# WujiangXu/AMID

Measured on AMD Instinct MI355X. Metric: train samples/sec, higher is better.
Workload: dtype f32; 1 GPU; cloth_sport_train75-shaped SASRec train step (BASELINE.json configs[1]); batch_per_gpu=256, global_batch=256, seq_len=50, emb_dim=128, hid_dim=32, neg=1, table_rows=894820, unique_rows_last_step=2102, input=HBM-resident batch pool, dropout=on (p=0.5), optimizer=Adam (dense-equivalent lazy rows), graph=True, steps_per_graph=1, parallelism=dp1

## Files before the change

amid_amd/csrc/sasrec_strip.hip:

```cpp
#include "common.h"
#include "rng.h"
#include "strip_gemm.h"
#include "strip_chain.h"
#include "sort_phases.h"
#include "attention_mfma.h"
#include "seq_bwd.h"
#include "scorer_sum.h"
#include <type_traits>

namespace amid {

struct StripQkvArgs {
    const float* x;
    const float* ln_w[2]; const float* ln_b[2];
    const float* w_in[2]; const float* b_in[2];
    float* qn; float* q; float* k; float* v;
    float ln_eps;
};

struct StripOffArgs {
    const float* o; const float* qn;
    const float* w_o[2]; const float* b_o[2]; const float* ln_w[2]; const float* ln_b[2];
    const float* w1[2]; const float* b1[2]; const float* w2[2]; const float* b2[2];
    const unsigned char* tmq;
    float* r; float* y; float* h; float* xo;
    float ln_eps;
    const StepState* st; int train; unsigned spec; float scale; int layer;
};

template <int D, bool XSTORE>
__device__ __forceinline__ void qkv_fwd_chain(const StripQkvArgs& a, const StripGeom& sg, Ring<D>& ring, const StripRow& row, int g,
                                              const StripRegs<D>& X, const ColVec<D>& lw, const ColVec<D>& lb) {
    constexpr int NT = D / 16;
    const GBuf gx(a.x, sg.act_bytes), gqn(a.qn, sg.act_bytes), gq(a.q, sg.act_bytes), gk(a.k, sg.act_bytes), gv(a.v, sg.act_bytes);
    StripRegs<D> Qn, Kr, Vr;
    ColVec<D> bias;
    strip_layernorm<D>(Qn, X, lw, lb, a.ln_eps);
    STRIP_STAMP(3);
    f32x4 acc[NT];
    {
        const float* buf = ring.next();
        STRIP_STAMP(4);
        bias.load(a.b_in[g] + D);
        strip_zero<D>(acc);
        strip_mma<D>(acc, X, buf, [&](int ct, int j) {
            ring.fetch(a.w_in[g] + 2LL * D * D, ct, j);
            if constexpr (XSTORE) store_spread<D>(gx, row, X, ct, j);
            store_spread<D>(gqn, row, Qn, ct, j);
        });
        STRIP_STAMP(5);
        add_bias<D>(acc, bias);
        to_regs<D>(Kr, acc);
        STRIP_STAMP(6);
    }
    {
        const float* buf = ring.next();
        STRIP_STAMP(7);
        bias.load(a.b_in[g] + 2 * D);
        strip_zero<D>(acc);
        strip_mma<D>(acc, X, buf, [&](int ct, int j) { ring.fetch(a.w_in[g], ct, j); store_spread<D>(gk, row, Kr, ct, j); });
        STRIP_STAMP(8);
        add_bias<D>(acc, bias);
        to_regs<D>(Vr, acc);
    }
    {
        const float* buf = ring.next();
        STRIP_STAMP(9);
        bias.load(a.b_in[g]);
        strip_zero<D>(acc);
        strip_mma<D>(acc, Qn, buf, [&](int ct, int j) { store_spread<D>(gv, row, Vr, ct, j); });
        STRIP_STAMP(10);
        add_bias<D>(acc, bias);
        to_regs<D>(Kr, acc);
        strip_store<D>(gq, row, Kr);
        STRIP_STAMP(11);
    }
}

template <int D>
__global__ __launch_bounds__(STRIP_THREADS) void strip_qkv_fwd_kernel(const StripQkvArgs a, const StripGeom sg) {
    extern __shared__ __attribute__((aligned(16))) float smem[];
    STRIP_STAMP(0);
    Ring<D> ring(smem);
    ring.first(a.w_in[strip_domain(blockIdx.x)] + 1LL * D * D);
    const StripTile t = strip_tile(sg, blockIdx.x);
    if (!t.live) { w_ring_wait(); return; }
    const StripRow row = strip_row<D>(sg, t);
    STRIP_STAMP(1);
    StripRegs<D> X;
    ColVec<D> lw, lb;
    strip_load<D>(X, GBuf(a.x, sg.act_bytes), row);
    lw.load(a.ln_w[t.g]); lb.load(a.ln_b[t.g]);
    STRIP_STAMP(2);
    qkv_fwd_chain<D, false>(a, sg, ring, row, t.g, X, lw, lb);
}

struct StripGatherArgs { const float* table; const int* idx; const float* pos[2]; unsigned char* tmq; };

template <int D>
__global__ __launch_bounds__(STRIP_THREADS) void strip_qkv_fwd_gather_kernel(const StripQkvArgs a, const StripGatherArgs ga, const StripGeom sg) {
    extern __shared__ __attribute__((aligned(16))) float smem[];
    Ring<D> ring(smem);
    ring.first(a.w_in[strip_domain(blockIdx.x)] + 1LL * D * D);
    const StripTile t = strip_tile(sg, blockIdx.x);
    if (!t.live) { w_ring_wait(); return; }
    const StripRow row = strip_row<D>(sg, t);
    StripRegs<D> X;
    ColVec<D> lw, lb;
    {
        const int gq = lane_id() >> 4;
        const int id = ga.idx[(long long)t.g * sg.M + row.local];
        const float* __restrict__ trow = ga.table + (long long)id * D;
        const float* __restrict__ prow = ga.pos[t.g] + (long long)(row.local % sg.T) * D;
        const GBuf gtm(ga.tmq, sg.tm_bytes);
        const unsigned tbase = row.ok ? (row.off - 16u * (unsigned)gq) >> 4 : STRIP_OOB;
#pragma unroll
        for (int ct = 0; ct < D / 16; ++ct) {
            const int col = ct * 16 + 4 * gq;
            const float4 tv = ld4_global(trow + col), pv = ld4_global(prow + col);
            float4 x = make_float4(tv.x + pv.x, tv.y + pv.y, tv.z + pv.z, tv.w + pv.w);
            const unsigned bits = (x.x == 0.f ? 1u : 0u) | (x.y == 0.f ? 2u : 0u) | (x.z == 0.f ? 4u : 0u) | (x.w == 0.f ? 8u : 0u);
            if (bits & 1u) x.x = 0.f;
            if (bits & 2u) x.y = 0.f;
            if (bits & 4u) x.z = 0.f;
            if (bits & 8u) x.w = 0.f;
            X.v[ct] = row.ok ? f32x4{x.x, x.y, x.z, x.w} : f32x4{0.f, 0.f, 0.f, 0.f};
            __builtin_amdgcn_raw_buffer_store_b8((unsigned char)bits, gtm.r, row.ok ? (int)(tbase + (unsigned)(ct * 4 + gq)) : (int)STRIP_OOB, 0, 0);
        }
    }
    lw.load(a.ln_w[t.g]); lb.load(a.ln_b[t.g]);
    qkv_fwd_chain<D, false>(a, sg, ring, row, t.g, X, lw, lb);
}

template <int D, bool NEXT, bool SAVE = true>
__global__ __launch_bounds__(STRIP_THREADS) void strip_oproj_ffn_fwd_kernel(const StripOffArgs a, const StripQkvArgs nx, const StripGeom sg) {
    extern __shared__ __attribute__((aligned(16))) float smem[];
    constexpr int NT = D / 16;
    Ring<D> ring(smem);
    ring.first(a.w_o[strip_domain(blockIdx.x)]);
    const StripTile t = strip_tile(sg, blockIdx.x);
    if (!t.live) { w_ring_wait(); return; }
    const StripRow row = strip_row<D>(sg, t);
    const int g = t.g;
    unsigned long long seed = 0; unsigned step = 0;
    if (a.train) { seed = a.st->seed; step = (unsigned)a.st->step; }
    const GBuf gr(a.r, sg.act_bytes), gy(a.y, sg.act_bytes), gh(a.h, sg.act_bytes), gxo(a.xo, sg.act_bytes);
    StripRegs<D> A, R, Y, H;
    StripTm<D> tm;
    ColVec<D> bias, lw, lb;
    strip_load<D>(A, GBuf(a.o, sg.act_bytes), row);
    strip_load<D>(R, GBuf(a.qn, sg.act_bytes), row);
    const bool has_tm = a.tmq != nullptr;
    if (has_tm) strip_tm_load<D>(tm, GBuf(a.tmq, sg.tm_bytes), row);
    bias.load(a.b_o[g]); lw.load(a.ln_w[g]); lb.load(a.ln_b[g]);
    f32x4 acc[NT];
    {
        const float* buf = ring.next();
        strip_zero<D>(acc);
        strip_mma<D>(acc, A, buf, [&](int ct, int j) { ring.fetch(a.w1[g], ct, j); });
        add_bias<D>(acc, bias);
// ... 327 lines not shown
        if (l == 0) strip_store<D>(GBuf(P.a.dx, sg.act_bytes), row, DX);
        DZ = DX;
    }
    STRIP_RSTAMP(13);
    STRIP_STAMP(15);
    w_ring_wait();
}

}

using namespace amid;
using namespace amid_strip_host;

static int make_rider(SortRider& rd, const void* sort_plan, int sort_phase) {
    rd.phase = 0;
    if (sort_plan == nullptr) return AMID_OK;
    if (sort_phase < 1 || sort_phase > 4) return AMID_ERR_ARG;
    rd.plan = *(const SortPlan*)sort_plan;
    rd.phase = sort_phase;
    return AMID_OK;
}

template <auto KERNEL, int DVAL, class... Args>
static int launch_strip_rider(const StripGeom& sg, const SortRider& rd, int extra, void* stream, const Args&... args) {
    if (rd.phase != 0 && strip_lds_bytes<DVAL>() < (rd.plan.g0.bits > 10 ? sizeof(SortScatterLds<OS_BINS_MAX>) : sizeof(SortScatterLds<1024>))) return AMID_ERR_UNSUPPORTED;
    return launch_lds<KERNEL>(2 * sg.tpg + rider_blocks_host(rd) + extra, STRIP_THREADS, strip_lds_bytes<DVAL>(), stream, args..., sg, rd);
}

extern "C" int amid_sas_strip_tile_rows(void) { return STRIP_TILE; }

#ifdef AMID_STRIP_STAMPS
extern "C" int amid_strip_stamps_read(unsigned long long* host) {
    return (int)hipMemcpyFromSymbol(host, HIP_SYMBOL(amid::amid_strip_stamp_buf), sizeof(unsigned long long) * STRIP_STAMP_WAVES * 32);
}
#endif

static void fill_strip_qkv(StripQkvArgs& a, const float* x, const float* const* ln_w, const float* const* ln_b, const float* const* w_in,
                           const float* const* b_in, float ln_eps, float* qn, float* q, float* k, float* v) {
    a.x = x; a.qn = qn; a.q = q; a.k = k; a.v = v; a.ln_eps = ln_eps;
    for (int g = 0; g < 2; ++g) { a.ln_w[g] = ln_w[g]; a.ln_b[g] = ln_b[g]; a.w_in[g] = w_in[g]; a.b_in[g] = b_in[g]; }
}

extern "C" int amid_sas_strip_qkv_fwd_f32(const float* x, const float* const* ln_w, const float* const* ln_b, const float* const* w_in,
                                          const float* const* b_in, float ln_eps, int B, int T, int D, const int* live, float* qn, float* q,
                                          float* k, float* v, void* stream) {
    AMID_CHECK_ARG(x && ln_w && ln_b && w_in && b_in && qn && q && k && v);
    StripQkvArgs a;
    fill_strip_qkv(a, x, ln_w, ln_b, w_in, b_in, ln_eps, qn, q, k, v);
    StripGeom sg;
    if (int e = make_strip_geom(B, T, D, live, &sg)) return e;
    if (D == 128) return launch_strip<strip_qkv_fwd_kernel<128>, 128>(sg, stream, a);
    if (D == 64) return launch_strip<strip_qkv_fwd_kernel<64>, 64>(sg, stream, a);
    return AMID_ERR_UNSUPPORTED;
}

struct StripOffCall {
    const float* o = nullptr; const float* qn = nullptr;
    FamC w_o = nullptr, b_o = nullptr, ln_w = nullptr, ln_b = nullptr, w1 = nullptr, b1 = nullptr, w2 = nullptr, b2 = nullptr;
    const unsigned char* tmq = nullptr; float ln_eps = 0.f;
    int B = 0, T = 0, D = 0; const int* live = nullptr; void* stream = nullptr;
    int layer = 0; const void* step_state = nullptr; int train = 0; float p_drop = 0.f;
    float* r = nullptr; float* y = nullptr; float* h = nullptr; float* xo = nullptr;
    FamC nln_w = nullptr, nln_b = nullptr, nw_in = nullptr, nb_in = nullptr;
    float* nqn = nullptr; float* nq = nullptr; float* nk = nullptr; float* nv = nullptr;
    bool save = true;
    bool next() const { return nln_w != nullptr; }
    bool next_operands() const { return nln_b && nw_in && nb_in && nqn && nq && nk && nv; }
};
#define STRIP_OFF_CALL(c)                                                                                                                       \
    StripOffCall c;                                                                                                                             \
    c.o = o; c.qn = qn; c.w_o = w_o; c.b_o = b_o; c.ln_w = ln_w; c.ln_b = ln_b; c.w1 = w1; c.b1 = b1; c.w2 = w2; c.b2 = b2; c.tmq = tmq;             \
    c.ln_eps = ln_eps; c.B = B; c.T = T; c.D = D; c.live = live; c.stream = stream; c.xo = xo; c.nln_w = nln_w; c.nln_b = nln_b; c.nw_in = nw_in;   \
    c.nb_in = nb_in; c.nqn = nqn; c.nq = nq; c.nk = nk; c.nv = nv

template <int D, bool SAVE>
static int launch_oproj_ffn_fwd(const StripGeom& sg, void* stream, bool next, const StripOffArgs& a, const StripQkvArgs& nx) {
    return next ? launch_strip<strip_oproj_ffn_fwd_kernel<D, true, SAVE>, D>(sg, stream, a, nx)
                : launch_strip<strip_oproj_ffn_fwd_kernel<D, false, SAVE>, D>(sg, stream, a, nx);
}
static int strip_oproj_ffn_fwd(const StripOffCall& c) {
    const bool next = c.next();
    StripOffArgs a;
    a.o = c.o; a.qn = c.qn; a.tmq = c.tmq; a.r = c.r; a.y = c.y; a.h = c.h; a.xo = c.xo; a.ln_eps = c.ln_eps;
    a.st = (const StepState*)c.step_state; a.layer = c.layer;
    const DropoutArgs d = dropout_args(c.train, c.p_drop);
    a.train = d.train; a.spec = d.spec; a.scale = d.scale;
    for (int g = 0; g < 2; ++g) {
        a.w_o[g] = c.w_o[g]; a.b_o[g] = c.b_o[g]; a.ln_w[g] = c.ln_w[g]; a.ln_b[g] = c.ln_b[g];
        a.w1[g] = c.w1[g]; a.b1[g] = c.b1[g]; a.w2[g] = c.w2[g]; a.b2[g] = c.b2[g];
    }
    StripQkvArgs nx = {};
    if (next) fill_strip_qkv(nx, c.save ? c.xo : nullptr, c.nln_w, c.nln_b, c.nw_in, c.nb_in, c.ln_eps, c.nqn, c.nq, c.nk, c.nv);
    StripGeom sg;
    if (int e = make_strip_geom(c.B, c.T, c.D, c.live, &sg)) return e;
    if (c.D == 128) return c.save ? launch_oproj_ffn_fwd<128, true>(sg, c.stream, next, a, nx) : launch_oproj_ffn_fwd<128, false>(sg, c.stream, next, a, nx);
    if (c.D == 64) return c.save ? launch_oproj_ffn_fwd<64, true>(sg, c.stream, next, a, nx) : launch_oproj_ffn_fwd<64, false>(sg, c.stream, next, a, nx);
    return AMID_ERR_UNSUPPORTED;
}

extern "C" int amid_sas_strip_oproj_ffn_fwd_f32(const float* o, const float* qn, const float* const* w_o, const float* const* b_o,
                                                const float* const* ln_w, const float* const* ln_b, const float* const* w1,
                                                const float* const* b1, const float* const* w2, const float* const* b2,
                                                const unsigned char* tmq, float ln_eps, int B, int T, int D, const int* live, int layer,
                                                const void* step_state, int train, float p_drop, float* r, float* y, float* h, float* xo,
                                                const float* const* nln_w, const float* const* nln_b, const float* const* nw_in,
                                                const float* const* nb_in, float* nqn, float* nq, float* nk, float* nv, void* stream) {
    STRIP_OFF_CALL(c); c.layer = layer; c.step_state = step_state; c.train = train; c.p_drop = p_drop; c.r = r; c.y = y; c.h = h;
    AMID_CHECK_ARG(o && qn && w_o && b_o && ln_w && ln_b && w1 && b1 && w2 && b2 && r && y && h && xo && (!train || step_state));
    AMID_CHECK_ARG(!c.next() || c.next_operands());
    return strip_oproj_ffn_fwd(c);
}

extern "C" int amid_sas_strip_infer_supported(int T, int D) { return (T > 0 && (D == 128 || D == 64)) ? 1 : 0; }

extern "C" int amid_sas_strip_qkv_fwd_gather_infer_f32(const float* table, const int* idx_all, const float* pos0, const float* pos1,
                                                       const float* const* ln_w, const float* const* ln_b, const float* const* w_in,
                                                       const float* const* b_in, float ln_eps, int B, int T, int D, const int* live,
                                                       unsigned char* tmq, float* qn, float* q, float* k, float* v, void* stream) {
    AMID_CHECK_ARG(table && idx_all && pos0 && pos1 && ln_w && ln_b && w_in && b_in && tmq && qn && q && k && v && B > 0 && T > 0 && D > 0);
    for (int g = 0; g < 2; ++g) AMID_CHECK_ARG(ln_w[g] && ln_b[g] && w_in[g] && b_in[g]);
    if (!amid_sas_strip_infer_supported(T, D)) return AMID_ERR_UNSUPPORTED;
    StripQkvArgs a;
    fill_strip_qkv(a, nullptr, ln_w, ln_b, w_in, b_in, ln_eps, qn, q, k, v);
    StripGatherArgs ga;
    ga.table = table; ga.idx = idx_all; ga.pos[0] = pos0; ga.pos[1] = pos1; ga.tmq = tmq;
    StripGeom sg;
    if (int e = make_strip_geom(B, T, D, live, &sg)) return e;
    if (D == 128) return launch_strip<strip_qkv_fwd_gather_kernel<128>, 128>(sg, stream, a, ga);
    return launch_strip<strip_qkv_fwd_gather_kernel<64>, 64>(sg, stream, a, ga);
}

extern "C" int amid_sas_strip_oproj_ffn_fwd_infer_f32(const float* o, const float* qn, const float* const* w_o, const float* const* b_o,
                                                      const float* const* ln_w, const float* const* ln_b, const float* const* w1,
                                                      const float* const* b1, const float* const* w2, const float* const* b2,
                                                      const unsigned char* tmq, float ln_eps, int B, int T, int D, const int* live, float* xo,
                                                      const float* const* nln_w, const float* const* nln_b, const float* const* nw_in,
                                                      const float* const* nb_in, float* nqn, float* nq, float* nk, float* nv, void* stream) {
    STRIP_OFF_CALL(c); c.save = false;
    AMID_CHECK_ARG(o && qn && w_o && b_o && ln_w && ln_b && w1 && b1 && w2 && b2 && B > 0 && T > 0 && D > 0);
    AMID_CHECK_ARG(c.next() ? c.next_operands() : xo != nullptr);
    for (int g = 0; g < 2; ++g) {
        AMID_CHECK_ARG(w_o[g] && b_o[g] && ln_w[g] && ln_b[g] && w1[g] && b1[g] && w2[g] && b2[g]);
        AMID_CHECK_ARG(!c.next() || (nln_w[g] && nln_b[g] && nw_in[g] && nb_in[g]));
    }
    if (!amid_sas_strip_infer_supported(T, D)) return AMID_ERR_UNSUPPORTED;
    return strip_oproj_ffn_fwd(c);
}
#undef STRIP_OFF_CALL

struct StripBwdLaunch {
    int B = 0, T = 0, D = 0; const int* live = nullptr;
    const void* sort_plan = nullptr; int sort_phase = 0;
    int mma_bf16 = 0;
    void* stream = nullptr;
};
#define STRIP_BWD_LAUNCH(l) StripBwdLaunch l; l.B = B; l.T = T; l.D = D; l.live = live; l.mma_bf16 = mma_bf16; l.stream = stream
#define STRIP_BWD_RIDER(l) l.sort_plan = sort_plan; l.sort_phase = sort_phase

template <int D, int BF>
static int launch_ffn_bwd(const StripGeom& sg, const SortRider& rd, void* stream, const StripFfnBwdArgs& a) {
    return rd.phase ? launch_strip_rider<strip_ffn_bwd_kernel<D, 2, BF>, D>(sg, rd, 0, stream, a)
                    : launch_strip_rider<strip_ffn_bwd_kernel<D, 0, BF>, D>(sg, rd, 0, stream, a);
}
static int strip_ffn_bwd(const FfnBwdCall& c, const StripBwdLaunch& l) {
    AMID_CHECK_ARG(c.dxo && c.operands());
    const int D = l.D, mma_bf16 = l.mma_bf16;
    if (mma_bf16 && D != 128) return AMID_ERR_UNSUPPORTED;
    StripFfnBwdArgs a;
    fill_ffn_bwd(a, c);
    StripGeom sg;
    if (int e = make_strip_geom(l.B, l.T, D, l.live, &sg)) return e;
    SortRider rd;
    if (int e = make_rider(rd, l.sort_plan, l.sort_phase)) return e;
    if (rd.phase != 0 && rd.phase != 2) return AMID_ERR_UNSUPPORTED;
    if (D == 128) return mma_bf16 == 3 ? launch_ffn_bwd<128, 3>(sg, rd, l.stream, a) : mma_bf16 ? launch_ffn_bwd<128, 1>(sg, rd, l.stream, a)
                                                                                          : launch_ffn_bwd<128, 0>(sg, rd, l.stream, a);
    if (D == 64) return launch_ffn_bwd<64, 0>(sg, rd, l.stream, a);
    return AMID_ERR_UNSUPPORTED;
}

extern "C" int amid_sas_strip_ffn_bwd_f32(const float* dxo, const unsigned char* tmq, const float* h, const float* r, const float* const* ln_w,
                                          const float* const* w1T, const float* const* w2T, const float* const* woT, float ln_eps, int B, int T,
                                          int D, const int* live, int layer, const void* step_state, int train, float p_drop, float* dpre2,
                                          float* dpre1, float* dr, float* d_o, float* ln_part, int mma_bf16, void* stream) {
    AMID_FFN_BWD_CALL(c); STRIP_BWD_LAUNCH(l);
    return strip_ffn_bwd(c, l);
}

extern "C" int amid_sas_strip_ffn_bwd_sort_f32(const float* dxo, const unsigned char* tmq, const float* h, const float* r,
                                               const float* const* ln_w, const float* const* w1T, const float* const* w2T,
                                               const float* const* woT, float ln_eps, int B, int T, int D, const int* live, int layer,
                                               const void* step_state, int train, float p_drop, float* dpre2, float* dpre1, float* dr,
                                               float* d_o, float* ln_part, const void* sort_plan, int sort_phase, int mma_bf16, void* stream) {
    AMID_CHECK_ARG(sort_plan != nullptr);
    AMID_FFN_BWD_CALL(c); STRIP_BWD_LAUNCH(l); STRIP_BWD_RIDER(l);
    return strip_ffn_bwd(c, l);
}

struct StripQkvBwdCall {
    const float* dq = nullptr; const float* dk = nullptr; const float* dv = nullptr; const float* dr = nullptr; const float* x = nullptr;
    FamC ln_w = nullptr, wqT = nullptr, wkT = nullptr, wvT = nullptr;
    float ln_eps = 0.f; float* dx = nullptr; float* ln_part = nullptr;
    const void* step_state = nullptr; int train = 0;
    FfnBwdCall ffn;
    const unsigned char* emb_tmq = nullptr; float emb_p_drop = 0.f;
    const ScorerSum* scorer = nullptr;
};
#define STRIP_QKV_BWD_CALL(c)                                                                                                                   \
    StripQkvBwdCall c;                                                                                                                          \
    c.dq = dq; c.dk = dk; c.dv = dv; c.dr = dr; c.x = x; c.ln_w = ln_w; c.wqT = wqT; c.wkT = wkT; c.wvT = wvT; c.ln_eps = ln_eps;                   \
    c.ln_part = ln_part; c.step_state = step_state; c.train = train
#define STRIP_QKV_BWD_FFN(c)                                                                                                                    \
    c.ffn.tmq = tmq; c.ffn.h = fh; c.ffn.r = fr; c.ffn.ln_w = fln_w; c.ffn.w1T = fw1T; c.ffn.w2T = fw2T; c.ffn.woT = fwoT; c.ffn.layer = flayer;    \
    c.ffn.p_drop = p_drop; c.ffn.dpre2 = fdpre2; c.ffn.dpre1 = fdpre1; c.ffn.dr = fdr; c.ffn.d_o = fd_o; c.ffn.ln_part = fln_part

template <int D, bool FFN, int BF>
static int launch_qkv_bwd(const StripGeom& sg, const SortRider& rd, void* stream, const StripQkvBwdArgs& a, const StripFfnBwdArgs& f, const ScorerSum& ss) {
    if constexpr (FFN && D == 128 && (BF == 3 || BF == 1))
        if (!rd.phase && ss.nblk > 0) return launch_strip_rider<strip_qkv_bwd_kernel<D, FFN, -1, BF>, D>(sg, rd, ss.nblk, stream, a, f, ss);
    return rd.phase ? launch_strip_rider<strip_qkv_bwd_kernel<D, FFN, FFN ? 3 : 4, BF>, D>(sg, rd, ss.nblk, stream, a, f, ss)
                    : launch_strip_rider<strip_qkv_bwd_kernel<D, FFN, 0, BF>, D>(sg, rd, 0, stream, a, f, ss);
}
static int strip_qkv_bwd(const StripQkvBwdCall& c, const StripBwdLaunch& l) {
    AMID_CHECK_ARG(c.dq && c.dk && c.dv && c.dr && c.x && c.ln_w && c.wqT && c.wkT && c.wvT && c.ln_part);
    const int D = l.D, mma_bf16 = l.mma_bf16;
    if (mma_bf16 && D != 128) return AMID_ERR_UNSUPPORTED;
    const bool ffn = c.ffn.h != nullptr;
    FfnBwdCall fc = c.ffn;
    fc.dxo = nullptr; fc.ln_eps = c.ln_eps; fc.step_state = c.step_state; fc.train = c.train;
    AMID_CHECK_ARG(c.emb_tmq == nullptr || (!ffn && (!c.train || c.step_state)));
    AMID_CHECK_ARG(ffn || c.dx);
    AMID_CHECK_ARG(!ffn || fc.operands());
    StripQkvBwdArgs a;
    a.dq = c.dq; a.dk = c.dk; a.dv = c.dv; a.dr = c.dr; a.x = c.x; a.dx = c.dx; a.ln_part = c.ln_part; a.ln_eps = c.ln_eps;
    for (int g = 0; g < 2; ++g) { a.ln_w[g] = c.ln_w[g]; a.wqT[g] = c.wqT[g]; a.wkT[g] = c.wkT[g]; a.wvT[g] = c.wvT[g]; }
    const DropoutArgs ed = dropout_args(c.emb_tmq && c.train, c.emb_p_drop);
    a.emb_tmq = c.emb_tmq; a.emb_st = (const StepState*)c.step_state;
    a.emb_train = ed.train; a.emb_spec = ed.spec; a.emb_scale = ed.scale;
    StripFfnBwdArgs f = {};
    if (ffn) fill_ffn_bwd(f, fc);
    StripGeom sg;
    if (int e = make_strip_geom(l.B, l.T, D, l.live, &sg)) return e;
    SortRider rd;
    if (int e = make_rider(rd, l.sort_plan, l.sort_phase)) return e;
    if (rd.phase != 0 && rd.phase != (ffn ? 3 : 4)) return AMID_ERR_UNSUPPORTED;
    ScorerSum ss = {};
    if (c.scorer != nullptr) {
        if (!(ffn && D == 128 && (mma_bf16 == 3 || mma_bf16 == 1))) return AMID_ERR_UNSUPPORTED;
        ss = *c.scorer;
    }
    void* const st = l.stream;
    if (D == 128 && mma_bf16 == 3) return ffn ? launch_qkv_bwd<128, true, 3>(sg, rd, st, a, f, ss) : launch_qkv_bwd<128, false, 3>(sg, rd, st, a, f, ss);
    if (D == 128 && mma_bf16) return ffn ? launch_qkv_bwd<128, true, 1>(sg, rd, st, a, f, ss) : launch_qkv_bwd<128, false, 1>(sg, rd, st, a, f, ss);
    if (D == 128) return ffn ? launch_qkv_bwd<128, true, 0>(sg, rd, st, a, f, ss) : launch_qkv_bwd<128, false, 0>(sg, rd, st, a, f, ss);
    if (D == 64) return ffn ? launch_qkv_bwd<64, true, 0>(sg, rd, st, a, f, ss) : launch_qkv_bwd<64, false, 0>(sg, rd, st, a, f, ss);
    return AMID_ERR_UNSUPPORTED;
}

extern "C" int amid_sas_strip_qkv_bwd_f32(const float* dq, const float* dk, const float* dv, const float* dr, const float* x,
                                          const float* const* ln_w, const float* const* wqT, const float* const* wkT, const float* const* wvT,
                                          float ln_eps, int B, int T, int D, const int* live, float* dx, float* ln_part,
                                          const unsigned char* tmq, const float* fh, const float* fr, const float* const* fln_w,
                                          const float* const* fw1T, const float* const* fw2T, const float* const* fwoT, int flayer,
                                          const void* step_state, int train, float p_drop, float* fdpre2, float* fdpre1, float* fdr,
                                          float* fd_o, float* fln_part, int mma_bf16, void* stream) {
    STRIP_QKV_BWD_CALL(c); STRIP_QKV_BWD_FFN(c); c.dx = dx; STRIP_BWD_LAUNCH(l);
    return strip_qkv_bwd(c, l);
}

extern "C" int amid_sas_strip_qkv_bwd_sort_f32(const float* dq, const float* dk, const float* dv, const float* dr, const float* x,
                                               const float* const* ln_w, const float* const* wqT, const float* const* wkT,
                                               const float* const* wvT, float ln_eps, int B, int T, int D, const int* live, float* dx,
                                               float* ln_part, const unsigned char* tmq, const float* fh, const float* fr,
                                               const float* const* fln_w, const float* const* fw1T, const float* const* fw2T,
                                               const float* const* fwoT, int flayer, const void* step_state, int train, float p_drop,
                                               float* fdpre2, float* fdpre1, float* fdr, float* fd_o, float* fln_part, const void* sort_plan,
                                               int sort_phase, int mma_bf16, void* stream) {
    AMID_CHECK_ARG(sort_plan != nullptr);
    STRIP_QKV_BWD_CALL(c); STRIP_QKV_BWD_FFN(c); c.dx = dx; STRIP_BWD_LAUNCH(l); STRIP_BWD_RIDER(l);
    return strip_qkv_bwd(c, l);
}

extern "C" int amid_sas_strip_qkv_bwd_sort_scorer_f32(const float* dq, const float* dk, const float* dv, const float* dr, const float* x,
                                                      const float* const* ln_w, const float* const* wqT, const float* const* wkT,
                                                      const float* const* wvT, float ln_eps, int B, int T, int D, const int* live,
                                                      float* ln_part, const unsigned char* tmq, const float* fh, const float* fr,
                                                      const float* const* fln_w, const float* const* fw1T, const float* const* fw2T,
                                                      const float* const* fwoT, int flayer, const void* step_state, int train, float p_drop,
                                                      float* fdpre2, float* fdpre1, float* fdr, float* fd_o, float* fln_part,
                                                      const void* sort_plan, int sort_phase, int mma_bf16, const float* hidg, const float* u,
                                                      const float* items, int NI, int hid, float* dW1, float* db1, float* dW2, float* db2,
                                                      void* stream) {
    AMID_CHECK_ARG(sort_plan != nullptr && fh != nullptr && hidg && u && items && NI > 0 && hid > 0 && dW1 && db1 && dW2 && db2);
    AMID_CHECK_ARG(((((unsigned long long)dW1) | ((unsigned long long)u) | ((unsigned long long)items)) & 15) == 0);
    const ScorerSum ss = scorer_sum_args(hidg, u, items, B, NI, D, hid, dW1, db1, dW2, db2);
    STRIP_QKV_BWD_CALL(c); STRIP_QKV_BWD_FFN(c); c.scorer = &ss; STRIP_BWD_LAUNCH(l); STRIP_BWD_RIDER(l);
    return strip_qkv_bwd(c, l);
}

extern "C" int amid_sas_strip_qkv_bwd_scorer_f32(const float* dq, const float* dk, const float* dv, const float* dr, const float* x,
                                                 const float* const* ln_w, const float* const* wqT, const float* const* wkT,
                                                 const float* const* wvT, float ln_eps, int B, int T, int D, const int* live,
                                                 float* ln_part, const unsigned char* tmq, const float* fh, const float* fr,
                                                 const float* const* fln_w, const float* const* fw1T, const float* const* fw2T,
                                                 const float* const* fwoT, int flayer, const void* step_state, int train, float p_drop,
                                                 float* fdpre2, float* fdpre1, float* fdr, float* fd_o, float* fln_part, int mma_bf16,
                                                 const float* hidg, const float* u, const float* items, int NI, int hid, float* dW1, float* db1,
                                                 float* dW2, float* db2, void* stream) {
    AMID_CHECK_ARG(fh != nullptr && hidg && u && items && NI > 0 && hid > 0 && dW1 && db1 && dW2 && db2);
    AMID_CHECK_ARG(((((unsigned long long)dW1) | ((unsigned long long)u) | ((unsigned long long)items)) & 15) == 0);
    const ScorerSum ss = scorer_sum_args(hidg, u, items, B, NI, D, hid, dW1, db1, dW2, db2);
    STRIP_QKV_BWD_CALL(c); STRIP_QKV_BWD_FFN(c); c.scorer = &ss; STRIP_BWD_LAUNCH(l);
    return strip_qkv_bwd(c, l);
}

extern "C" int amid_sas_strip_qkv_bwd_emb_f32(const float* dq, const float* dk, const float* dv, const float* dr, const float* x,
                                              const float* const* ln_w, const float* const* wqT, const float* const* wkT,
                                              const float* const* wvT, float ln_eps, int B, int T, int D, const int* live, float* dx,
                                              float* ln_part, const unsigned char* emb_tmq, const void* step_state, int train,
                                              float emb_p_drop, const void* sort_plan, int sort_phase, int mma_bf16, void* stream) {
    AMID_CHECK_ARG(emb_tmq != nullptr && dx != nullptr);
    STRIP_QKV_BWD_CALL(c); c.dx = dx; c.emb_tmq = emb_tmq; c.emb_p_drop = emb_p_drop; STRIP_BWD_LAUNCH(l); STRIP_BWD_RIDER(l);
    return strip_qkv_bwd(c, l);
}
#undef AMID_FFN_BWD_CALL
#undef STRIP_QKV_BWD_FFN
#undef STRIP_QKV_BWD_CALL
#undef STRIP_BWD_RIDER
#undef STRIP_BWD_LAUNCH

template <int D> static constexpr size_t seq_bwd_lds_bytes() { return strip_lds_bytes<D>() + (size_t)STRIP_WAVES * ATTN_BWD_LDS_PER_WAVE; }

extern "C" int amid_sas_seq_bwd_supported(int B, int T, int D, int H) {
    return ((D == 128 || D == 64) && H == 8 && T > 0 && T <= 64 && B > 0 && 2LL * B * T * D * 4 <= 0x7FFFFFF0LL) ? 1 : 0;
}

extern "C" int amid_diag_variants(void) {
#ifdef AMID_DIAG_VARIANTS
    return 1;
#else
    return 0;
#endif
}
static int g_seq_bwd_variant = 0;
extern "C" int amid_sas_seq_bwd_variant(int v) {
    const int prev = g_seq_bwd_variant;
    if (v >= 0) g_seq_bwd_variant = v;
    return prev;
}

extern "C" int amid_sas_seq_bwd_f32(int n_layers, const float* dxo, const unsigned char* tmq, const float* const* h, const float* const* r,
                                    const float* const* x, const float* const* q, const float* const* k, const float* const* v,
                                    const float* const* o, const float* const* stats, const float* const* ln1_w,
                                    const float* const* ln2_w, const float* const* wqT, const float* const* wkT, const float* const* wvT,
                                    const float* const* woT, const float* const* w1T, const float* const* w2T, float ln_eps, int B, int T,
                                    int D, int H, const int* live, const void* step_state, int train, float p_drop, float* const* dpre2,
                                    float* const* dpre1, float* const* dr, float* d_o, float* const* dq, float* const* dk, float* const* dv,
                                    float* dx, float* const* ln1_part, float* const* ln2_part, int mma_bf16, void* stream) {
    AMID_CHECK_ARG(n_layers >= 1 && n_layers <= 2 && dxo && h && r && x && q && k && v && o && stats && ln1_w && ln2_w && wqT && wkT && wvT &&
                   woT && w1T && w2T && live && dpre2 && dpre1 && dr && d_o && dq && dk && dv && dx && ln1_part && ln2_part &&
                   (!train || step_state));
    if (!amid_sas_seq_bwd_supported(B, T, D, H)) return AMID_ERR_UNSUPPORTED;
    SeqBwdArgs a = {};
    a.n_layers = n_layers;
    for (int l = 0; l < n_layers; ++l) {
        SeqBwdLayer& P = a.L[l];
        AMID_CHECK_ARG(h[l] && r[l] && x[l] && q[l] && k[l] && v[l] && o[l] && stats[l] && dpre2[l] && dpre1[l] && dr[l] && dq[l] && dk[l] &&
                       dv[l] && ln1_part[l] && ln2_part[l]);
        for (int g = 0; g < 2; ++g) {
            const int i = 2 * l + g;
            AMID_CHECK_ARG(ln1_w[i] && ln2_w[i] && wqT[i] && wkT[i] && wvT[i] && woT[i] && w1T[i] && w2T[i]);
        }
        FfnBwdCall fc;
        fc.dxo = l + 1 == n_layers ? dxo : nullptr; fc.tmq = tmq; fc.h = h[l]; fc.r = r[l]; fc.ln_w = ln2_w + 2 * l; fc.w1T = w1T + 2 * l;
        fc.w2T = w2T + 2 * l; fc.woT = woT + 2 * l; fc.ln_eps = ln_eps; fc.layer = l; fc.step_state = step_state; fc.train = train; fc.p_drop = p_drop;
        fc.dpre2 = dpre2[l]; fc.dpre1 = dpre1[l]; fc.dr = dr[l]; fc.d_o = d_o; fc.ln_part = ln2_part[l];
        fill_ffn_bwd(P.f, fc);
        P.a.dq = dq[l]; P.a.dk = dk[l]; P.a.dv = dv[l]; P.a.dr = dr[l]; P.a.x = x[l]; P.a.dx = l == 0 ? dx : nullptr;
        P.a.ln_part = ln1_part[l]; P.a.ln_eps = ln_eps;
        for (int g = 0; g < 2; ++g) {
            P.a.ln_w[g] = ln1_w[2 * l + g]; P.a.wqT[g] = wqT[2 * l + g]; P.a.wkT[g] = wkT[2 * l + g]; P.a.wvT[g] = wvT[2 * l + g];
        }
        AttnArgs& at = P.at;
        at.q = q[l]; at.k = k[l]; at.v = v[l]; at.o = const_cast<float*>(o[l]); at.stats = const_cast<float*>(stats[l]);
        at.d_o = d_o; at.dq = dq[l]; at.dk = dk[l]; at.dv = dv[l];
        at.B = B; at.T = T; at.D = D; at.H = H; at.causal = 1; at.layer = l;
        at.scale = sqrtf(1.0f / (float)(D / H));
        at.st = (const StepState*)step_state;
        const DropoutArgs ad = dropout_args(train, p_drop);
        at.train = ad.train; at.thr16 = ad.spec; at.dscale = ad.scale;
        at.stagger_from = -1;
    }
    StripGeom sg;
    if (int e = make_strip_geom(B, T, D, live, &sg)) return e;
    if (g_seq_bwd_variant == 2 || T <= 32 || D != 128) {
        const int rc = launch_seqn_bwd(a, sg, D, mma_bf16, stream);
        if (rc != AMID_ERR_UNSUPPORTED || T <= 32 || D != 128) return rc;
    }
    return mma_bf16 ? launch_lds<seq_bwd_kernel<128, true>>(B, STRIP_THREADS, seq_bwd_lds_bytes<128>(), stream, a, sg)
                    : launch_lds<seq_bwd_kernel<128, false>>(B, STRIP_THREADS, seq_bwd_lds_bytes<128>(), stream, a, sg);
}
```

amid_amd/csrc/sasrec_strip_px.hip:

```cpp
#include "common.h"
#include "rng.h"
#include "strip_gemm.h"
#include "strip_chain.h"
#include "seq_fwd.h"
#include "seq_bwd.h"
#include "seqn_parts.h"
#include "sort_phases.h"

namespace amid {

constexpr int PXB_WPS = 4, PXB_NS = 2, PXB_NW = PXB_WPS * PXB_NS, PXB_THREADS = 64 * PXB_NW;
template <int D> constexpr size_t pxb_lds_floats() {
    return (size_t)3 * (D * D / 2) + (size_t)PXB_WPS * XpStrip<D>::FLOATS + 2 * PXB_NW * 16 + (size_t)PXB_WPS * 2 * D;
}

struct PxbRow { unsigned off_own, phys; int local; bool ok; };
template <int D>
__device__ __forceinline__ PxbRow pxb_row(const StripGeom& sg, const StripTile& t, int si, int c0) {
    PxbRow r;
    int v = t.v0 + si * 16 + (lane_id() & 15);
    r.ok = v < t.nv;
    if (!r.ok) v = t.v0;
    if (sg.live != nullptr) {
        const int s = v / sg.T;
        r.local = sg.live[t.s0 + s] * sg.T + (v - s * sg.T);
    } else {
        r.local = v;
    }
    r.phys = (unsigned)t.g * (unsigned)sg.M + (unsigned)r.local;
    r.off_own = r.ok ? r.phys * (unsigned)(D * 4) + 16u * (unsigned)(lane_id() >> 4) + (unsigned)c0 * 64u : STRIP_OOB;
    return r;
}

template <int NCT>
__device__ __forceinline__ void pxb_row_sums(float* __restrict__ stat, int si, int part, float s1, float s2, float& t1, float& t2) {
    const int m = lane_id() & 15, gq = lane_id() >> 4;
    s1 = row_sum4(s1); s2 = row_sum4(s2);
    if (gq == 0) {
        lds_st1(stat + (si * PXB_NS + part) * 16 + m, s1);
        lds_st1(stat + (PXB_NW + si * PXB_NS + part) * 16 + m, s2);
    }
    lds_barrier();
    t1 = 0.f; t2 = 0.f;
#pragma unroll
    for (int p = 0; p < PXB_NS; ++p) {
        t1 += *(__attribute__((address_space(3))) float*)(stat + (si * PXB_NS + p) * 16 + m);
        t2 += *(__attribute__((address_space(3))) float*)(stat + (PXB_NW + si * PXB_NS + p) * 16 + m);
    }
}

template <int D, int NCT>
__device__ __forceinline__ void pxb_ln_partials(float* __restrict__ scratch, int si, int c0, const PartRegs<NCT>& dgam, const PartRegs<NCT>& dbet) {
    const int lane = lane_id();
    float* mine = scratch + si * 2 * D;
#pragma unroll
    for (int c = 0; c < NCT; ++c) {
        f32x4 a, b;
#pragma unroll
        for (int r = 0; r < 4; ++r) { a[r] = col_sum16(dgam.v[c][r]); b[r] = col_sum16(dbet.v[c][r]); }
        if ((lane & 15) == 0) {
            lds_st4(mine + (c0 + c) * 16 + 4 * (lane >> 4), a);
            lds_st4(mine + D + (c0 + c) * 16 + 4 * (lane >> 4), b);
        }
    }
}
template <int D>
__device__ __forceinline__ void pxb_ln_partials_out(const float* __restrict__ scratch, float* __restrict__ part) {
    for (int e = threadIdx.x; e < 2 * D; e += PXB_THREADS)
        part[e] = (scratch[e] + scratch[2 * D + e]) + (scratch[4 * D + e] + scratch[6 * D + e]);
}

template <int D, int NCT, class Ring>
__device__ __forceinline__ void pxb_ffn_bwd_chain(const StripFfnBwdArgs& a, const float* __restrict__ ln_stat, const StripGeom& sg, Ring& ring,
                                                  const PxbRow& row, int g, int si, int part, int c0, PartRegs<NCT>& DZ, float* __restrict__ xps,
                                                  float* __restrict__ stat, float* __restrict__ lnsc, const unsigned short* __restrict__ wnext) {
    const int lane = lane_id(), gq = lane >> 4;
    const GBuf gp2(a.dpre2, sg.act_bytes), gp1(a.dpre1, sg.act_bytes), gdr(a.dr, sg.act_bytes), gdo(a.d_o, sg.act_bytes);
    PartRegs<NCT> P, Hs, Rs, gam;
    part_load<NCT>(Hs, GBuf(a.h, sg.act_bytes), row.off_own);
    part_load<NCT>(Rs, GBuf(a.r, sg.act_bytes), row.off_own);
    part_cols<NCT>(gam, a.ln_w[g], c0);
    float mean = 0.f, rstd = 0.f;
    if (ln_stat != nullptr && row.ok) { mean = ln_stat[(long long)row.phys * 4 + 2]; rstd = ln_stat[(long long)row.phys * 4 + 3]; }
    if (a.tmq != nullptr) {
        const GBuf gtm(a.tmq, sg.tm_bytes);
        const unsigned tbase = row.ok ? row.phys * (unsigned)(D / 4) + (unsigned)c0 * 4u : STRIP_OOB;
        const int sh = 8 * gq;
#pragma unroll
        for (int c = 0; c < NCT; ++c) {
            const unsigned bits = (unsigned)__builtin_amdgcn_raw_buffer_load_b32(gtm.r, (int)(tbase + 4 * c), 0, 0) >> sh;
            DZ.v[c][0] = (bits & 1u) ? 0.f : DZ.v[c][0];
            DZ.v[c][1] = (bits & 2u) ? 0.f : DZ.v[c][1];
            DZ.v[c][2] = (bits & 4u) ? 0.f : DZ.v[c][2];
            DZ.v[c][3] = (bits & 8u) ? 0.f : DZ.v[c][3];
        }
    }
    P = DZ;
    if (a.train) {
        const uint4 rr2 = rng_call(a.st->seed, (unsigned long long)row.local * D >> 7, site_id(g, a.layer, SITE_FFN2), (unsigned)a.st->step);
        part_dropout<NCT>(P, rr2, c0, a.spec, a.scale, (row.local * D) & 127);
    }
    xp_write<NCT>(xps, c0, P);
    f32x4 acc[NCT];
    {
        ring.next();
        seqn_product_xp<D, NCT>(acc, xps, ring, (const unsigned short*)a.w1T[g], c0, [&](int ct, int j) { part_spread<NCT>(gp2, row.off_own, P, ct, j, 1); });
#pragma unroll
        for (int c = 0; c < NCT; ++c)
#pragma unroll
            for (int r = 0; r < 4; ++r) P.v[c][r] = Hs.v[c][r] > 0.f ? acc[c][r] * a.scale : 0.f;
    }
    lds_barrier();
    xp_write<NCT>(xps, c0, P);
    PartRegs<NCT> DR, dgam, dbet;
    {
        ring.next();
        seqn_product_xp<D, NCT>(acc, xps, ring, (const unsigned short*)a.woT[g], c0, [&](int ct, int j) { part_spread<NCT>(gp1, row.off_own, P, ct, j, 1); });
        if (ln_stat == nullptr) {
            float sm = 0.f;
#pragma unroll
            for (int c = 0; c < NCT; ++c) sm += (Rs.v[c][0] + Rs.v[c][1]) + (Rs.v[c][2] + Rs.v[c][3]);
            float tot, dummy;
            pxb_row_sums<NCT>(stat, si, part, sm, 0.f, tot, dummy);
            mean = tot * (1.0f / D);
            float q = 0.f;
#pragma unroll
            for (int c = 0; c < NCT; ++c)
#pragma unroll
                for (int r = 0; r < 4; ++r) { const float d = Rs.v[c][r] - mean; q = fmaf(d, d, q); }
            lds_barrier();
            float qt;
            pxb_row_sums<NCT>(stat, si, part, q, 0.f, qt, dummy);
            rstd = 1.0f / sqrtf(qt * (1.0f / D) + a.ln_eps);
            lds_barrier();
        }
        float s1 = 0.f, s2 = 0.f;
#pragma unroll
        for (int c = 0; c < NCT; ++c) {
#pragma unroll
            for (int r = 0; r < 4; ++r) {
                const float dy = acc[c][r] + DZ.v[c][r];
                const float xh = (Rs.v[c][r] - mean) * rstd;
                float gy = gam.v[c][r] * dy;
                asm volatile("" : "+v"(gy));
                s1 += gy;
                s2 = fmaf(gy, xh, s2);
                float dg = dy * xh;
                asm volatile("" : "+v"(dg));
                dgam.v[c][r] = dg;
                dbet.v[c][r] = dy;
                DR.v[c][r] = gy;
            }
        }
        float t1, t2;
        pxb_row_sums<NCT>(stat, si, part, s1, s2, t1, t2);
        const float c1 = t1 * (1.0f / D), c2 = t2 * (1.0f / D);
#pragma unroll
        for (int c = 0; c < NCT; ++c)
#pragma unroll
            for (int r = 0; r < 4; ++r) {
                const float xh = (Rs.v[c][r] - mean) * rstd;
                DR.v[c][r] = rstd * (DR.v[c][r] - c1 - xh * c2);
            }
    }
    xp_write<NCT>(xps, c0, DR);
    {
        ring.next();
        seqn_product_xp<D, NCT>(acc, xps, ring, wnext, c0, [&](int ct, int j) { part_spread<NCT>(gdr, row.off_own, DR, ct, j, 1); });
#pragma unroll
        for (int c = 0; c < NCT; ++c) P.v[c] = acc[c];
        part_store<NCT>(gdo, row.off_own, P);
    }
    pxb_ln_partials<D, NCT>(lnsc, si, c0, dgam, dbet);
}

template <int D, int RIDER>
__global__ __launch_bounds__(PXB_THREADS) void strip_ffn_bwd_px_kernel(const StripFfnBwdArgs a, const float* __restrict__ ln_stat, const StripGeom sg,
                                                                       const SortRider rd) {
    extern __shared__ __attribute__((aligned(16))) float smem[];
    constexpr int NCT = D / 16 / PXB_NS;
    int bid = blockIdx.x;
    if constexpr (RIDER != 0) {
        if (bid < rd.plan.nblk) { if (threadIdx.x < SORT_THREADS) sort_phase_ct<RIDER>(rd.plan, bid, smem); return; }
        bid -= rd.plan.nblk;
    }
    const int w = wave_id(), part = w / PXB_WPS, si = w % PXB_WPS, c0 = part * NCT;
    const int g = strip_domain(bid);
    SeqRing3<D, PXB_NW> ring(smem);
    ring.first((const unsigned short*)a.w2T[g]);
    const StripTile t = strip_tile(sg, bid);
    if (!t.live) { zero_slot<D>(a.ln_part, t.slot); w_ring_wait(); return; }
    float* const xps = smem + 3 * SeqRing3<D, PXB_NW>::SLAB + si * XpStrip<D>::FLOATS;
    float* const stat = smem + 3 * SeqRing3<D, PXB_NW>::SLAB + PXB_WPS * XpStrip<D>::FLOATS;
    float* const lnsc = stat + 2 * PXB_NW * 16;
    const PxbRow row = pxb_row<D>(sg, t, si, c0);
    PartRegs<NCT> DZ;
    part_load<NCT>(DZ, GBuf(a.dxo, sg.act_bytes), row.off_own);
    pxb_ffn_bwd_chain<D, NCT>(a, ln_stat, sg, ring, row, g, si, part, c0, DZ, xps, stat, lnsc, (const unsigned short*)a.woT[g]);
    w_ring_wait();
    __syncthreads();
    pxb_ln_partials_out<D>(lnsc, a.ln_part + (long long)t.slot * 2 * D);
}

}

using namespace amid;
using namespace amid_strip_host;

extern "C" int amid_sas_strip_ffn_bwd_px_f32(const float* dxo, const unsigned char* tmq, const float* h, const float* r, const float* const* ln_w,
                                             const float* const* w1T, const float* const* w2T, const float* const* woT, float ln_eps, int B, int T,
                                             int D, const int* live, int layer, const void* step_state, int train, float p_drop, float* dpre2,
                                             float* dpre1, float* dr, float* d_o, float* ln_part, const float* ln_stat, const void* sort_plan,
                                             int sort_phase, void* stream) {
    AMID_FFN_BWD_CALL(c);
    AMID_CHECK_ARG(c.dxo && c.operands());
    if (D != 128) return AMID_ERR_UNSUPPORTED;
    if (train && p_drop > 0.f && spec_bits(drop_spec(p_drop)) != 1) return AMID_ERR_UNSUPPORTED;
    StripGeom sg;
    if (int e = make_strip_geom(B, T, D, live, &sg)) return e;
    StripFfnBwdArgs a;
    fill_ffn_bwd(a, c);
    SortRider rd;
    rd.phase = 0;
    if (sort_plan != nullptr) {
        if (sort_phase != 2) return AMID_ERR_UNSUPPORTED;
        rd.plan = *(const SortPlan*)sort_plan;
        rd.phase = sort_phase;
    }
    constexpr size_t lds = pxb_lds_floats<128>() * sizeof(float);
    static_assert(lds >= sizeof(SortScatterLds<OS_BINS_MAX>), "the rider's scatter fits the head of the allocation");
    if (rd.phase != 0) return launch_lds<strip_ffn_bwd_px_kernel<128, 2>>(2 * sg.tpg + rd.plan.nblk, PXB_THREADS, lds, stream, a, ln_stat, sg, rd);
    return launch_lds<strip_ffn_bwd_px_kernel<128, 0>>(2 * sg.tpg, PXB_THREADS, lds, stream, a, ln_stat, sg, rd);
}
#undef AMID_FFN_BWD_CALL
```

amid_amd/engine.py:

```python
from __future__ import annotations

import ctypes
import types
from dataclasses import dataclass
from typing import Dict, List, Optional, Tuple

import torch

from ._lib import lib, ptr_array

from .engine_dp import DataParallelMixin, HipMergeBackend
from .engine_graph import GraphMixin
from .engine_io import InputMixin
from .engine_topk import TopkMixin
from .plan import (DR_HEADS, SASREC_HEADS, SASREC_LN_EPS, SASREC_P_DROP, FlatParams, SasrecPlan, Shape,
                   sasrec_dense_names)

SASREC_FAMILIES = (("ln1_w", "attention_layernorms.{l}.weight"), ("ln1_b", "attention_layernorms.{l}.bias"),
                   ("w_in", "attention_layers.{l}.in_proj_weight"), ("b_in", "attention_layers.{l}.in_proj_bias"),
                   ("w_o", "attention_layers.{l}.out_proj.weight"), ("b_o", "attention_layers.{l}.out_proj.bias"),
                   ("ln2_w", "forward_layernorms.{l}.weight"), ("ln2_b", "forward_layernorms.{l}.bias"),
                   ("w1", "forward_layers.{l}.conv1.weight"), ("b1", "forward_layers.{l}.conv1.bias"),
                   ("w2", "forward_layers.{l}.conv2.weight"), ("b2", "forward_layers.{l}.conv2.bias"))
QKV_FAMILIES = tuple(n for n, _ in SASREC_FAMILIES[:4])
# ... 58 lines not shown
        self._push_step_state()
        self.plans: Dict[Tuple[int, int, int, bool], SasrecPlan] = {}
        self.grad_scale = 1.0
        self.opt_bank, self._banks = 0, {}
        torch.cuda.synchronize(self.device)
        self._ptr_cache: Dict[str, object] = {}

    @property
    def s(self) -> int:
        return self.stream.cuda_stream

    def sync(self) -> None:
        self.join_sort()
        self.stream.synchronize()

    def _push_step_state(self) -> None:
        L = lib()
        host = (ctypes.c_ubyte * self._st_bytes)()
        L.call("amid_step_state_pack", ctypes.addressof(host), self.seed, self.step, self.hyper["lr"], self.hyper["beta1"],
               self.hyper["beta2"], self.hyper["eps"])
        with torch.cuda.stream(self.stream):
            self.step_state.copy_(torch.frombuffer(bytearray(host), dtype=torch.uint8), non_blocking=False)

    @staticmethod
    def rank_seed(seed: int, rank: int) -> int:
        return (int(seed) + 0x9E3779B97F4A7C15 * int(rank)) & 0x7FFFFFFFFFFFFFFF

    def set_step(self, step: int, seed: Optional[int] = None) -> None:
        self.step = int(step)
        if seed is not None:
            self.seed = int(seed)
        self._push_step_state()

    def set_lr(self, lr: float) -> None:
        self.hyper["lr"] = float(lr)
        self._push_step_state()

    def _ensure_opt_state(self) -> None:
        if self.table_m is None:
            self.table_m = torch.zeros_like(self.table)
            self.table_v = torch.zeros_like(self.table)
            self.table_last = torch.zeros(self.n_rows, dtype=torch.int32, device=self.device)
            torch.cuda.synchronize(self.device)

    def select_optimizer(self, k: int, lr: Optional[float] = None) -> None:
        if k == self.opt_bank:
            if lr is not None and lr != self.hyper["lr"]:
                self.set_lr(lr)
            return
        self.flush_table()
        self.sync()
        fp = self.dense
        self._banks[self.opt_bank] = dict(m=fp.m, v=fp.v, tm=self.table_m, tv=self.table_v, tl=self.table_last, st=self.step_state,
                                          step=self.step, lr=self.hyper["lr"], seed=self.seed)
        b = self._banks.get(k)
        if b is None:
            b = dict(m=torch.zeros_like(fp.m), v=torch.zeros_like(fp.v), tm=None, tv=None, tl=None,
                     st=torch.empty(self._st_bytes, dtype=torch.uint8, device=self.device), step=0,
                     lr=self.hyper["lr"] if lr is None else float(lr), seed=self.seed + 0x9E3779B9 * k)
        fp.m, fp.v, self.table_m, self.table_v, self.table_last = b["m"], b["v"], b["tm"], b["tv"], b["tl"]
        self.step_state, self.step, self.seed = b["st"], b["step"], b["seed"]
        self.hyper["lr"] = b["lr"] if lr is None else float(lr)
        self.opt_bank = k
        self._push_step_state()
        torch.cuda.synchronize(self.device)

    def _graph_key(self) -> Tuple[int, int]:
        return (self.opt_bank, self.dr_mode if self.dr else 0)

    def plan(self, B: int, T: int, NI: int, need_grad: bool) -> SasrecPlan:
        key = (B, T, NI, need_grad)
        if key not in self.plans:
            inc = getattr(self, "inc_bs", 0)
            if (2 * T if inc else T) > self.Tpos:
                raise ValueError(f"sequence length {T} exceeds pos_emb size {self.Tpos}" + (" / 2 (isInC)" if inc else ""))
            self.plans[key] = self.PLAN_CLS(self, Shape(B, T, NI, 2 * T if inc else 0), need_grad)
            torch.cuda.synchronize(self.device)
        return self.plans[key]

    def _pp(self, fmt: str, buf: Optional[torch.Tensor] = None, extra: int = 0):
        return self._cached((fmt, 0 if buf is None else buf.data_ptr(), extra),
                            lambda: ptr_array([self.dense.ptr(fmt.format(d=d), buf, extra) for d in (1, 2)]))

    def _wT(self, layer: int, which: int):
        bf = self._bf16_bwd
        p3 = self._p3_bwd
        return self._cached(("wT16x3" if p3 else "wT16" if bf else "wT", layer, which), lambda: ptr_array(
            [(self.wT16x3 if p3 else self.wT16 if bf else self.wT)[layer, g, which].data_ptr() for g in (0, 1)]))

    def _cached(self, key, build):
        c = self._ptr_cache.get(key)
        if c is None:
            c = self._ptr_cache[key] = build()
        return c

    def _fams(self):
        fp = self.dense
        return self._cached("fams", lambda: {n: ptr_array([fp.ptr(f"sac{d}." + fmt.format(l=l)) for l in (0, 1) for d in (1, 2)])
                                             for n, fmt in SASREC_FAMILIES})

    def _lay(self):
        return self._cached("lay", lambda: [{n: self._pp("sac{d}." + fmt.format(l=l)) for n, fmt in SASREC_FAMILIES} for l in (0, 1)])

    def _pos(self):
        fp = self.dense
        return self._cached("pos", lambda: dict(pos0=fp.ptr("sac1.pos_emb.weight"), pos1=fp.ptr("sac2.pos_emb.weight")))

    def _scorer(self, names=("w1", "b1", "w2", "b2"), grad: bool = False):
        fp = self.dense
        return self._cached(("scorer", names, grad), lambda: dict(zip(names, (
            fp.ptr("predictModule.fc." + n, fp.grad if grad else None) for n in ("0.weight", "0.bias", "2.weight", "2.bias")))))

    def _last_ln(self, names=("ln_w", "ln_b")):
        return self._cached(("last_ln", names), lambda: dict(zip(names, (self._pp("sac{d}.last_layernorm.weight"),
                                                                          self._pp("sac{d}.last_layernorm.bias")))))

    def _wT_fams(self, bf16: bool):
        buf = self.wT16 if bf16 else self.wT
        return self._cached(("wT_fams", bool(bf16)), lambda: {
            n: ptr_array([buf[l, g, j].data_ptr() for l in (0, 1) for g in (0, 1)]) for j, n in enumerate(("wqT", "wkT", "wvT", "woT", "w1T", "w2T"))})

    def _wT_lists(self):
        def build():
            fp, D, src, dst = self.dense, self.D, [], []
            for l in (0, 1):
                for g in (0, 1):
                    pre = f"sac{g + 1}"
                    src += [fp.ptr(f"{pre}.attention_layers.{l}.in_proj_weight", None, j * D * D) for j in range(3)]
                    src += [fp.ptr(f"{pre}.attention_layers.{l}.out_proj.weight"), fp.ptr(f"{pre}.forward_layers.{l}.conv1.weight"),
                            fp.ptr(f"{pre}.forward_layers.{l}.conv2.weight")]
                    dst += [self.wT[l, g, w].data_ptr() for w in range(6)]
            return ptr_array(src), ptr_array(dst), len(src)
        return self._cached("wT_lists", build)

    @staticmethod
    def _seq_ptrs(pl: SasrecPlan):
        if not hasattr(pl, "seq_ptrs"):
            pa = lambda ts: ptr_array([t.data_ptr() for t in ts])
            pl.seq_ptrs = dict(x_in=pa(pl.x[:2]), qn=pa(pl.qn), q=pa(pl.q), k=pa(pl.k), v=pa(pl.v), o=pa(pl.o), stats=pa(pl.stats), r=pa(pl.r),
                               y=pa(pl.y), h=pa(pl.h))
        return pl.seq_ptrs

    @staticmethod
    def _seq_grad_ptrs(pl: SasrecPlan):
        if not hasattr(pl, "seq_grad_ptrs"):
            pa = lambda ts: ptr_array([t.data_ptr() for t in ts])
            pl.seq_grad_ptrs = dict(dpre2=pa(pl.dpre2), dpre1=pa(pl.dpre1), dr=pa(pl.dr), dq=pa(pl.dq_l), dk=pa(pl.dk_l), dv=pa(pl.dv_l),
                                    ln1_part=pa(pl.ln1_part_s), ln2_part=pa(pl.ln2_part_s))
        return pl.seq_grad_ptrs

    _bf16_bwd = False
    _p3_bwd = False
    BWD_SPLIT = True

    def enqueue_prepare(self, pl: SasrecPlan, sparse: bool, bump_step: bool = False, defer_sort: bool = False) -> None:
        L, s, shp = lib(), self.s, pl.shape
        with_live = bool(bump_step and getattr(pl, "strip", False) and not self.itc_bs)
        pl.live_packed = with_live
        pl.compact = bool(with_live and sparse and self.compact_ok(pl))
        pl.riding = bool(bump_step and sparse and defer_sort and self.SORT_RIDERS and getattr(pl, "strip", False) and not pl.compact
                         and not self._seq_backward(pl)
                         and (shp.n_idx + 2047) // 2048 <= 2 * shp.Tenc and self._sort_plan(pl) is not None)
        pl.chain = bool(bump_step and sparse and defer_sort and self.SORT_CHAIN and not pl.riding and not pl.compact
                        and shp.n_idx <= lib().value("amid_sort_chain_max_indices") and self.n_rows <= (1 << 20) and self._sort_plan(pl) is not None)
        ent = self.input_pool(pl)
        self._bf16_as_f32 = False
        if self.compute == "bf16" and self.BF16_FOLD and bump_step and shp.B <= self.BF16_FOLD_MAX_B:
            self._bf16_as_f32 = True
            if not (ent is not None and sparse and defer_sort and with_live and self._tail2_ok(pl)):
                self._bf16_as_f32 = False
            else:
                pl.riding = False
        pl.tail2 = bool(ent is not None and bump_step and sparse and defer_sort and with_live and self._tail2_ok(pl))
        pl.gather_on_fwd = False
        pl.prepared = False
        if pl.tail2:
            pool, phase = ent
            self._ensure_opt_state()
            head = (pool.data_ptr(), pool.stride(0), pool.shape[0], phase, pl.in_pack.data_ptr(), pl.in_words, shp.B, shp.T,
                    shp.NI - 1, self.n_rows, pl.idx_all.data_ptr(), pl.idx_c.data_ptr(), pl.row_c.data_ptr(), pl.live.data_ptr(), pl.err.data_ptr(),
                    self.table.data_ptr(), self.table_m.data_ptr(), self.table_v.data_ptr(), self.table_last.data_ptr(), self.D,
                    self.step_state.data_ptr(), self._sort_plan_c(pl))
            pl.gather_on_fwd = bool(self.GATHER_ON_FWD and self._fwd_on_pieces(pl, shp.B, shp.Tenc) and self._p3_bwd_for(pl) and shp.T == shp.Tenc)
            slabs = self.pool_slabs(pl)
            pl.prepared = bool(self.PREPARED_POOL and slabs is not None and getattr(self, "_in_train_step", False) and self.compute != "bf16")
            if pl.prepared:
                w = (None, 0, 0, None, None)
                if pl.gather_on_fwd:
                    src, w16 = self._w16_images(3)
                    w = (src, 24, 3, w16.data_ptr(), self._wT16x3_buf().data_ptr())
                L.call("amid_step_head_prepared_f32", *head, slabs[0].data_ptr(), slabs[0].stride(0), *w, s)
            elif pl.gather_on_fwd:
                src, w16 = self._w16_images(3)
                L.call("amid_step_head_w16_f32", *head, src, 24, 3, w16.data_ptr(), self._wT16x3_buf().data_ptr(), s)
            else:
                L.call("amid_step_head_f32", *head, s)
            self.step += 1
            pl.compact, pl.riding, pl.chain = True, not pl.prepared, False
            self._sort_owed = False
            return
        if ent is not None:
            pool, phase = ent
            if not bump_step:
                raise ValueError("an input pool advances with the step counter: enqueue_prepare(bump_step=True) only")
            if with_live:
                L.call("amid_pack_indices_pool_live", pool.data_ptr(), pool.stride(0), pool.shape[0], phase, pl.in_pack.data_ptr(),
                       pl.in_words, shp.B, shp.T, shp.NI - 1, self.n_rows, pl.idx_all.data_ptr(), pl.err.data_ptr(),
                       self.step_state.data_ptr(), pl.live.data_ptr(), s)
            else:
                L.call("amid_pack_indices_pool", pool.data_ptr(), pool.stride(0), pool.shape[0], phase, pl.in_pack.data_ptr(),
                       pl.in_words, shp.B, shp.T, shp.NI - 1, self.n_rows, pl.idx_all.data_ptr(), pl.err.data_ptr(),
                       self.step_state.data_ptr(), s)
            self.step += 1
            if sparse and (pl.riding or pl.chain):
                self._sort_owed = False
            elif sparse:
                self.ev_idx.record(self.stream)
                self._sort_owed = bool(defer_sort)
                if not defer_sort:
                    self.enqueue_sort(pl)
            return
        if with_live:
            L.call("amid_pack_indices_live", pl.in_i_node.data_ptr(), pl.in_neg.data_ptr(), pl.in_seq_d1.data_ptr(), pl.in_seq_d2.data_ptr(),
                   shp.B, shp.T, shp.NI - 1, self.n_rows, pl.idx_all.data_ptr(), pl.err.data_ptr(),
                   self.step_state.data_ptr() if bump_step else None, pl.domain.data_ptr(), pl.live.data_ptr(), s)
        else:
            L.call("amid_pack_indices", pl.in_i_node.data_ptr(), pl.in_neg.data_ptr(), pl.in_seq_d1.data_ptr(), pl.in_seq_d2.data_ptr(),
                   shp.B, shp.T, shp.NI - 1, self.n_rows, pl.idx_all.data_ptr(), pl.err.data_ptr(),
                   self.step_state.data_ptr() if bump_step else None, s)
        if bump_step:
            self.step += 1
        if sparse and (pl.riding or pl.chain):
            self._sort_owed = False
        elif sparse:
            self.ev_idx.record(self.stream)
            self._sort_owed = bool(defer_sort)
            if not defer_sort:
                self.enqueue_sort(pl)

    def enqueue_sort(self, pl: SasrecPlan) -> None:
        L, shp = lib(), pl.shape
        self.side.wait_event(self.ev_idx)
        if getattr(pl, "compact", False):
            L.call("amid_sort_unique_rows_i32", pl.idx_c.data_ptr(), pl.row_c.data_ptr(), pl.n_compact, self.n_rows, pl.sort_ws.data_ptr(),
                   pl.pos_sorted.data_ptr(), pl.uniq_ids.data_ptr(), pl.seg_off.data_ptr(), pl.seg_of.data_ptr(), pl.n_uniq.data_ptr(),
                   self.side.cuda_stream)
        else:
            L.call("amid_sort_unique_i32", pl.idx_all.data_ptr(), shp.n_idx, self.n_rows, pl.sort_ws.data_ptr(), pl.pos_sorted.data_ptr(),
                   pl.uniq_ids.data_ptr(), pl.seg_off.data_ptr(), pl.seg_of.data_ptr(), pl.n_uniq.data_ptr(), self.side.cuda_stream)
        self.ev_sorted.record(self.side)
        self._sort_pending = True
        self._sort_owed = False

    def _wgrad_mode(self, D: int) -> int:
        if D != 128:
            return 0
        if self.BF16_WGRAD and getattr(self, "_bf16_bwd", False):
            return 1
        if self._bf16_as_f32 and self.BF16_WGRAD and self.BF16_FWD_ONE and getattr(self, "_wgrad_one", False):
            return 4
        return {"9": 2, "6": 3}.get(self.WGRAD_SPLIT, 0)

    def join_sort(self) -> None:
        if getattr(self, "_sort_pending", False):
            self.stream.wait_event(self.ev_sorted)
            self._sort_pending = False

    SORT_RIDERS = True
    BF16_FOLD = True
    BF16_FOLD_MAX_B = 1 << 30
    BF16_FWD_ONE = True
    _bf16_as_f32 = False

    def _ceff(self) -> str:
        return "f32" if self._bf16_as_f32 else self.compute
    FOLD_SHORT = True
    SORT_CHAIN = False
    BF16_WGRAD = True
    WGRAD_SPLIT = "6"
    FWD_SPLIT = True
    SEQ_BACKWARD = "auto"

    def _seq_backward(self, pl: SasrecPlan) -> bool:
        if not getattr(pl, "seq_bwd", False) or self.itc_bs or self.SEQ_BACKWARD in ("0", False):
            return False
        if self.SEQ_BACKWARD in ("1", True):
            return True
        n_cu = torch.cuda.get_device_properties(self.device).multi_processor_count
        if pl.shape.Tenc <= 32:
            if self.FOLD_SHORT and pl.shape.Tenc > 16 and self.D == 128 and self._folded_step_shape(pl):
                return False
            return pl.shape.B <= n_cu
        if self.D != 128:
            return False
        if self._folded_step_shape(pl):
            return False
        return n_cu < pl.shape.B <= 2 * n_cu

    def _sort_plan(self, pl: SasrecPlan):
        if not hasattr(pl, "_sort_plan_buf"):
            L = lib()
            buf = (ctypes.c_ubyte * L.value("amid_sort_plan_bytes"))()
            rc = L._fn["amid_sort_plan_pack"](ctypes.addressof(buf), pl.idx_all.data_ptr(), None, pl.shape.n_idx, self.n_rows,
                                              pl.sort_ws.data_ptr(), pl.pos_sorted.data_ptr(), pl.uniq_ids.data_ptr(), pl.seg_off.data_ptr(),
                                              pl.seg_of.data_ptr(), pl.n_uniq.data_ptr())
            pl._sort_plan_buf = buf if rc == 0 else None
# ... 392 lines not shown
                pl.du_raw.copy_(pl.du_raw_g[:, ex.rank * B:(ex.rank + 1) * B])
                for d in (1, 2):
                    for name in ("trans_nn.weight", "trans_nn.bias", "trans_bs.weight", "trans_bs.bias"):
                        self.dense.view(f"itc_d{d}.{name}", G).mul_(1.0 / ex.world)
            du = pl.du_raw
        L.call("amid_lnmean_bwd_f32", pl.x[2].data_ptr(), du.data_ptr(), fp.ptr("sac1.last_layernorm.weight"),
               fp.ptr("sac2.last_layernorm.weight"), B, T, D, SASREC_LN_EPS, pl.dxbuf.data_ptr(), pl.last_part.data_ptr(), s)

    def _scorer_fwd(self, pl: SasrecPlan, head: str, items: int, p1, p2, with_loss: bool) -> None:
        shp, fp = pl.shape, self.dense
        lib().call("amid_scorer_fwd_f32", pl.u.data_ptr(), items, fp.ptr(f"{head}.fc.0.weight"), fp.ptr(f"{head}.fc.0.bias"),
                   fp.ptr(f"{head}.fc.2.weight"), fp.ptr(f"{head}.fc.2.bias"), pl.labels.data_ptr() if with_loss else None,
                   pl.domain.data_ptr() if with_loss else None, shp.B, shp.NI, self.D, self.hid, p1.data_ptr(), p2.data_ptr(),
                   pl.dp1.data_ptr() if with_loss else None, pl.dp2.data_ptr() if with_loss else None,
                   pl.loss_part.data_ptr() if with_loss else None, self.s)

    def _scorer_bwd(self, pl: SasrecPlan, head: str, items: int, ditems: int, p1, p2, dp1, dp2, part, accumulate: int) -> None:
        shp, fp = pl.shape, self.dense
        lib().call("amid_scorer_bwd_f32", pl.u.data_ptr(), items, fp.ptr(f"{head}.fc.0.weight"), fp.ptr(f"{head}.fc.0.bias"),
                   fp.ptr(f"{head}.fc.2.weight"), fp.ptr(f"{head}.fc.2.bias"), p1.data_ptr(), p2.data_ptr(), dp1.data_ptr(), dp2.data_ptr(),
                   shp.B, shp.NI, self.D, self.hid, pl.du.data_ptr(), ditems, part.data_ptr(), accumulate, self.s)

    def _enqueue_head_itc_fwd(self, pl: SasrecPlan, items: int, with_loss: bool) -> None:
        self._enqueue_user_vectors(pl)
        self._scorer_fwd(pl, "predictModule", items, pl.p1, pl.p2, with_loss)

    def _enqueue_head_itc_bwd(self, pl: SasrecPlan, items: int, ditems: int) -> None:
        self._scorer_bwd(pl, "predictModule", items, ditems, pl.p1, pl.p2, pl.dp1, pl.dp2, pl.sc_part, 0)
        self._enqueue_user_vectors_bwd(pl)

    def _enqueue_head_dr_fwd(self, pl: SasrecPlan, items: int, with_loss: bool) -> None:
        L, shp = lib(), pl.shape
        self._enqueue_user_vectors(pl)
        self._scorer_fwd(pl, "predictModule", items, pl.p1, pl.p2, False)
        self._scorer_fwd(pl, "predict_ips", items, pl.ips1, pl.ips2, False)
        self._scorer_fwd(pl, "predict_gfunc", items, pl.g1, pl.g2, False)
        if with_loss:
            pa = lambda a, b: ptr_array([a.data_ptr(), b.data_ptr()])
            L.call("amid_dr_loss_f32", pa(pl.p1, pl.p2), pa(pl.ips1, pl.ips2), pa(pl.g1, pl.g2), pl.labels.data_ptr(), pl.domain.data_ptr(),
                   pl.in_ob.data_ptr(), self.dr_mode, self.dr_e_w, shp.B, shp.NI, pa(pl.dp1, pl.dp2), pa(pl.dips1, pl.dips2),
                   pa(pl.dg1, pl.dg2), pl.dr_loss_part.data_ptr(), self.s)

    def _enqueue_head_dr_bwd(self, pl: SasrecPlan, items: int, ditems: int) -> None:
        self._scorer_bwd(pl, "predictModule", items, ditems, pl.p1, pl.p2, pl.dp1, pl.dp2, pl.sc_part, 0)
        self._scorer_bwd(pl, "predict_ips", items, ditems, pl.ips1, pl.ips2, pl.dips1, pl.dips2, pl.sc_part_ips, 1)
        self._scorer_bwd(pl, "predict_gfunc", items, ditems, pl.g1, pl.g2, pl.dg1, pl.dg2, pl.sc_part_g, 1)
        self._enqueue_user_vectors_bwd(pl)

    def _enqueue_scorers_fused(self, pl: SasrecPlan, items: int, ditems: int, tr_src, tr_dst, n_tr: int) -> None:
        shp, fp = pl.shape, self.dense
        heads = DR_HEADS if self.dr else DR_HEADS[:1]
        outs = [(pl.p1, pl.p2, pl.dp1, pl.dp2, pl.sc_part)]
        if self.dr:
            outs += [(pl.ips1, pl.ips2, pl.dips1, pl.dips2, pl.sc_part_ips), (pl.g1, pl.g2, pl.dg1, pl.dg2, pl.sc_part_g)]
        pa = lambda seq: ptr_array(list(seq))
        lib().call("amid_scorer_multi_fwd_bwd_f32", pl.u.data_ptr(), items, pa(fp.ptr(f"{h}.fc.0.weight") for h in heads),
                   pa(fp.ptr(f"{h}.fc.0.bias") for h in heads), pa(fp.ptr(f"{h}.fc.2.weight") for h in heads),
                   pa(fp.ptr(f"{h}.fc.2.bias") for h in heads), len(heads), pl.labels.data_ptr(), pl.domain.data_ptr(),
                   pl.in_ob.data_ptr() if self.dr else None, self.dr_mode if self.dr else 0, self.dr_e_w, shp.B, shp.NI, self.D, self.hid,
                   pa(o[0].data_ptr() for o in outs), pa(o[1].data_ptr() for o in outs), pa(o[2].data_ptr() for o in outs),
                   pa(o[3].data_ptr() for o in outs), pl.loss_part.data_ptr(), pl.dr_loss_part.data_ptr() if self.dr else None,
                   pl.du.data_ptr(), ditems, pa(o[4].data_ptr() for o in outs), tr_src, tr_dst, n_tr, self.s)

    def _head_io(self, pl: SasrecPlan, items: int, ditems: int):
        shp = pl.shape
        return dict(x=pl.x[2].data_ptr(), items=items, labels=pl.labels.data_ptr(), domain_id=pl.domain.data_ptr(), B=shp.B, T=shp.Tenc, NI=shp.NI,
                    D=self.D, hid=self.hid, eps=SASREC_LN_EPS, u=pl.u.data_ptr(), p1=pl.p1.data_ptr(), p2=pl.p2.data_ptr(), dp1=pl.dp1.data_ptr(),
                    dp2=pl.dp2.data_ptr(), loss_part=pl.loss_part.data_ptr(), dx=pl.dxbuf.data_ptr(), ditems=ditems,
                    ln_part=pl.last_part.data_ptr(), stream=self.s)

    def enqueue_backward(self, pl: SasrecPlan, train: bool) -> None:
        L, s, shp, D = lib(), self.s, pl.shape, self.D
        B, T, NI, M = shp.B, shp.Tenc, shp.NI, shp.M
        st = self.step_state.data_ptr()
        tr = 1 if train else 0
        fp = self.dense
        tr_src, tr_dst, n_tr = self._wT_lists()
        self._bf16_bwd = bool(self._ceff() == "bf16" and pl.strip)
        self._p3_bwd = self._p3_bwd_for(pl)
        bf = 3 if self._p3_bwd else 1 if self._bf16_bwd else 0
        if self._bf16_as_f32 and self._p3_bwd:
            bf = 1
        if self._bf16_bwd:
            if not hasattr(self, "wT16"):
                self.wT16 = torch.empty(2, 2, 6, D * D, dtype=torch.bfloat16, device=self.device)
            L.call("amid_sas_weights_bf16", tr_src, n_tr, D, 1, self.wT16.data_ptr(), s)
        if self._p3_bwd:
            if not getattr(pl, "wT16x3_written", False):
                L.call("amid_sas_weights_bf16_planes", tr_src, n_tr, D, 1, 3, self._wT16x3_buf().data_ptr(), s)
            pl.wT16x3_written = False
        items = pl.xg.data_ptr() + 4 * 2 * shp.Mi * D
        ditems = pl.dxg.data_ptr() + 4 * 2 * shp.Mi * D
        if (self.dr or self.itc_bs) and getattr(self, "_fuse_scorers", False):
            self._enqueue_scorers_fused(pl, items, ditems, tr_src, tr_dst, n_tr)
            self._enqueue_user_vectors_bwd(pl)
        elif self.dr:
            L.call("amid_transpose_weights_f32", tr_src, tr_dst, n_tr, D, s)
            self._enqueue_head_dr_bwd(pl, items, ditems)
        elif self.itc_bs:
            L.call("amid_transpose_weights_f32", tr_src, tr_dst, n_tr, D, s)
            self._enqueue_head_itc_bwd(pl, items, ditems)
        elif getattr(pl, "head_done", False):
            pl.head_done = False
        elif getattr(self, "_fuse_head", False) and getattr(pl, "tail2", False) and getattr(self, "_live_fwd", False) and self._live_list(pl) is not None:
            L.call_named("amid_head_fwd_bwd_own_vec_f32", self._last_ln(), self._scorer(), self._head_io(pl, items, ditems),
                         hidg=self._hidg(pl).data_ptr(), tr_src=None, tr_dst=None, n_tr=0)
        elif getattr(self, "_fuse_head", False):
            L.call_named("amid_head_fwd_bwd_own_f32" if getattr(self, "_live_fwd", False) and self._live_list(pl) is not None else "amid_head_fwd_bwd_f32",
                         self._last_ln(), self._scorer(), self._head_io(pl, items, ditems), sc_part=pl.sc_part.data_ptr(), tr_src=tr_src,
                         tr_dst=tr_dst, n_tr=n_tr)
        else:
            L.call_named("amid_head_bwd_f32", self._last_ln(), self._scorer(), x=pl.x[2].data_ptr(), u=pl.u.data_ptr(), items=items,
                         p1=pl.p1.data_ptr(), p2=pl.p2.data_ptr(), dp1=pl.dp1.data_ptr(), dp2=pl.dp2.data_ptr(), B=B, T=T, NI=NI, D=D,
                         hid=self.hid, eps=SASREC_LN_EPS, dx=pl.dxbuf.data_ptr(), ditems=ditems, ln_part=pl.last_part.data_ptr(),
                         sc_part=pl.sc_part.data_ptr(), tr_src=tr_src, tr_dst=tr_dst, n_tr=n_tr, stream=s)
        def ffn_bwd_args(l):
            return (pl.tmq.data_ptr(), pl.h[l].data_ptr(), pl.r[l].data_ptr(), self._pp(f"sac{{d}}.forward_layernorms.{l}.weight"),
                    self._wT(l, 4), self._wT(l, 5), self._wT(l, 3))

        lv = self._live_list(pl)
        live_attn = lv is not None and bool(lib().value("amid_attn_live_supported", T, D, self.H, 1))

        def attn_bwd(l):
            if live_attn:
                L.call("amid_attn_bwd_live_f32", pl.q[l].data_ptr(), pl.k[l].data_ptr(), pl.v[l].data_ptr(), pl.o[l].data_ptr(),
                       pl.stats[l].data_ptr(), pl.d_o.data_ptr(), B, T, D, self.H, 1, l, st, tr, SASREC_P_DROP, pl.dq_l[l].data_ptr(),
                       pl.dk_l[l].data_ptr(), pl.dv_l[l].data_ptr(), lv, s)
                return
            L.call("amid_attn_bwd_rows_f32", pl.q[l].data_ptr(), pl.k[l].data_ptr(), pl.v[l].data_ptr(), pl.o[l].data_ptr(),
                   pl.stats[l].data_ptr(), pl.d_o.data_ptr(), None, B, T, D, self.H, 1, l, st, tr, SASREC_P_DROP, pl.dq_l[l].data_ptr(),
                   pl.dk_l[l].data_ptr(), pl.dv_l[l].data_ptr(), self._own_rows(pl), s)

        dom = self._own_rows(pl)
        live = dom is not None and pl.live_rows
        tm, h1, r1, lnw1, w1T1, w2T1, woT1 = ffn_bwd_args(1)
        tm, h0, r0, lnw0, w1T0, w2T0, woT0 = ffn_bwd_args(0)
        dx_in = (pl.dx0 if self.inc_bs else pl.dxg).data_ptr()
        seq = bool(pl.strip and lv is not None and live and live_attn and self._seq_backward(pl))
        pl.seq_bwd_used = seq
        if seq:
            sv = self._seq_ptrs(pl)
            L.call_named("amid_sas_seq_bwd_f32", sv, self._seq_grad_ptrs(pl), self._fams(), self._wT_fams(bf), n_layers=2, dxo=pl.dxbuf.data_ptr(),
                         tmq=tm, x=sv["x_in"], ln_eps=SASREC_LN_EPS, B=B, T=T, D=D, H=self.H, live=lv, step_state=st, train=tr,
                         p_drop=SASREC_P_DROP, d_o=pl.d_o.data_ptr(), dx=dx_in, mma_bf16=bf, stream=s)
        elif pl.strip:
            ln1p, ln2p = pl.ln1_part, pl.ln2_part
            riding = getattr(pl, "riding", False)
            sfx = "_sort" if riding else ""
            t2 = getattr(pl, "tail2", False)
            plan_addr = (self._sort_plan_c(pl) if t2 else self._sort_plan(pl)) if riding else None
            ride = lambda ph: (plan_addr, ph) if riding else ()
            L.call(f"amid_sas_strip_ffn_bwd{sfx}_f32", pl.dxbuf.data_ptr(), tm, h1, r1, lnw1, w1T1, w2T1, woT1, SASREC_LN_EPS, B, T, D, lv, 1, st, tr,
                   SASREC_P_DROP, pl.dpre2[1].data_ptr(), pl.dpre1[1].data_ptr(), pl.dr[1].data_ptr(), pl.d_o.data_ptr(), ln2p[1].data_ptr(),
                   *ride(2), bf, s)
            attn_bwd(1)
            if t2:
                mid = ("amid_sas_strip_qkv_bwd_sort_scorer_f32", dict(sort_plan=plan_addr, sort_phase=3)) if riding else ("amid_sas_strip_qkv_bwd_scorer_f32", {})
                L.call_named(mid[0], self._scorer(("dW1", "db1", "dW2", "db2"), grad=True), **mid[1],
                             dq=pl.dq_l[1].data_ptr(), dk=pl.dk_l[1].data_ptr(), dv=pl.dv_l[1].data_ptr(), dr=pl.dr[1].data_ptr(),
                             x=pl.x[1].data_ptr(), ln_w=self._pp("sac{d}.attention_layernorms.1.weight"), wqT=self._wT(1, 0), wkT=self._wT(1, 1),
                             wvT=self._wT(1, 2), ln_eps=SASREC_LN_EPS, B=B, T=T, D=D, live=lv, ln_part=ln1p[1].data_ptr(), tmq=tm, fh=h0, fr=r0,
                             fln_w=lnw0, fw1T=w1T0, fw2T=w2T0, fwoT=woT0, flayer=0, step_state=st, train=tr, p_drop=SASREC_P_DROP,
                             fdpre2=pl.dpre2[0].data_ptr(), fdpre1=pl.dpre1[0].data_ptr(), fdr=pl.dr[0].data_ptr(), fd_o=pl.d_o.data_ptr(),
                             fln_part=ln2p[0].data_ptr(), mma_bf16=bf, hidg=self._hidg(pl).data_ptr(),
                             u=pl.u.data_ptr(), items=items, NI=NI, hid=self.hid, stream=s)
            else:
                L.call(f"amid_sas_strip_qkv_bwd{sfx}_f32", pl.dq_l[1].data_ptr(), pl.dk_l[1].data_ptr(), pl.dv_l[1].data_ptr(), pl.dr[1].data_ptr(),
                       pl.x[1].data_ptr(), self._pp("sac{d}.attention_layernorms.1.weight"), self._wT(1, 0), self._wT(1, 1), self._wT(1, 2),
                       SASREC_LN_EPS, B, T, D, lv, None, ln1p[1].data_ptr(), tm, h0, r0, lnw0, w1T0, w2T0, woT0, 0, st, tr, SASREC_P_DROP,
                       pl.dpre2[0].data_ptr(), pl.dpre1[0].data_ptr(), pl.dr[0].data_ptr(), pl.d_o.data_ptr(), ln2p[0].data_ptr(), *ride(3), bf, s)
            attn_bwd(0)
            if t2:
                L.call("amid_sas_strip_qkv_bwd_emb_f32", pl.dq_l[0].data_ptr(), pl.dk_l[0].data_ptr(), pl.dv_l[0].data_ptr(), pl.dr[0].data_ptr(),
                       pl.x[0].data_ptr(), self._pp("sac{d}.attention_layernorms.0.weight"), self._wT(0, 0), self._wT(0, 1), self._wT(0, 2),
                       SASREC_LN_EPS, B, T, D, lv, dx_in, ln1p[0].data_ptr(), pl.tmq.data_ptr(), st, tr, SASREC_P_DROP, plan_addr, 4 if riding else 0, bf, s)
            else:
                L.call(f"amid_sas_strip_qkv_bwd{sfx}_f32", pl.dq_l[0].data_ptr(), pl.dk_l[0].data_ptr(), pl.dv_l[0].data_ptr(), pl.dr[0].data_ptr(),
                       pl.x[0].data_ptr(), self._pp("sac{d}.attention_layernorms.0.weight"), self._wT(0, 0), self._wT(0, 1), self._wT(0, 2),
                       SASREC_LN_EPS, B, T, D, lv, dx_in, ln1p[0].data_ptr(), None, None, None, None, None, None, None, 0, None, 0, 0.0, None,
                       None, None, None, None, *ride(4), bf, s)
        else:
            rows, suf, rpt = ("_rows", pl.rt_suffix_v, pl.rpt_v) if live else ("", pl.rt_suffix, pl.rpt)
            ln1p, ln2p = (pl.ln1_part_v, pl.ln2_part_v) if live else (pl.ln1_part, pl.ln2_part)
            hint = (dom, B, T) if live else ()
            L.call(f"amid_sas_ffn_bwd{rows}_f32" + suf, pl.dxbuf.data_ptr(), tm, h1, r1, lnw1, w1T1, w2T1, woT1, SASREC_LN_EPS, M, D, rpt, 1, st, tr,
                   SASREC_P_DROP, pl.dpre2[1].data_ptr(), pl.dpre1[1].data_ptr(), pl.dr[1].data_ptr(), pl.d_o.data_ptr(),
                   ln2p[1].data_ptr(), self.mma_bf16, *hint, s)
            attn_bwd(1)
            L.call(f"amid_sas_qkv_ffn_bwd{rows}_f32" + suf, pl.dq_l[1].data_ptr(), pl.dk_l[1].data_ptr(), pl.dv_l[1].data_ptr(), pl.dr[1].data_ptr(),
                   pl.x[1].data_ptr(), self._pp("sac{d}.attention_layernorms.1.weight"), self._wT(1, 0), self._wT(1, 1), self._wT(1, 2),
                   SASREC_LN_EPS, M, D, rpt, pl.dxbuf.data_ptr(), ln1p[1].data_ptr(), tm, h0, r0, lnw0, w1T0, w2T0, woT0, 0, st, tr,
                   SASREC_P_DROP, pl.dpre2[0].data_ptr(), pl.dpre1[0].data_ptr(), pl.dr[0].data_ptr(), pl.d_o.data_ptr(),
                   ln2p[0].data_ptr(), self.mma_bf16, *hint, s)
            attn_bwd(0)
            L.call(f"amid_sas_qkv_bwd{rows}_f32" + suf, pl.dq_l[0].data_ptr(), pl.dk_l[0].data_ptr(), pl.dv_l[0].data_ptr(), pl.dr[0].data_ptr(),
                   pl.x[0].data_ptr(), self._pp("sac{d}.attention_layernorms.0.weight"), self._wT(0, 0), self._wT(0, 1), self._wT(0, 2),
                   SASREC_LN_EPS, M, D, rpt, dx_in, ln1p[0].data_ptr(), self.mma_bf16, *hint, s)
        dy, xx = [], []
        for l in (0, 1):
            dy += [pl.dq_l[l].data_ptr(), pl.dk_l[l].data_ptr(), pl.dv_l[l].data_ptr(), pl.dr[l].data_ptr(), pl.dpre1[l].data_ptr(),
                   pl.dpre2[l].data_ptr()]
            xx += [pl.qn[l].data_ptr(), pl.x[l].data_ptr(), pl.x[l].data_ptr(), pl.o[l].data_ptr(), pl.y[l].data_ptr(), pl.h[l].data_ptr()]
        t2 = bool(getattr(pl, "tail2", False) and pl.strip and not seq)
        if t2:
            if getattr(pl, "lnstat_fwd", False):
                for l in (0, 1):
                    xx[6 * l + 0], xx[6 * l + 4] = pl.x[l].data_ptr(), pl.r[l].data_ptr()
                self._wgrad_one = True
                try:
                    wmode = self._wgrad_mode(D)
                finally:
                    self._wgrad_one = False
                wg = ("amid_sas_wgrad_rows_sort_ln_f32", dict(sort_plan=self._sort_plan_c(pl))) if pl.riding else ("amid_sas_wgrad_rows_ln_f32", {})
                L.call_named(wg[0], self._fams(), dy=ptr_array(dy), x=ptr_array(xx), n_layers=2, M=M, D=D,
                             splits=pl.splits, w_part=ptr_array([pl.w_part[0].data_ptr(), pl.w_part[1].data_ptr()]),
                             b_part=ptr_array([pl.b_part[0].data_ptr(), pl.b_part[1].data_ptr()]), row_domain=self._own_rows(pl), B=B, T=T,
                             mma_bf16=wmode, ln_stat=self._ln_stat(pl)[1], stream=s, **wg[1])
            elif not pl.riding:
                L.call("amid_sas_wgrad_rows_f32", ptr_array(dy), ptr_array(xx), 2, M, D, pl.splits,
                       ptr_array([pl.w_part[0].data_ptr(), pl.w_part[1].data_ptr()]), ptr_array([pl.b_part[0].data_ptr(), pl.b_part[1].data_ptr()]),
                       self._own_rows(pl), B, T, self._wgrad_mode(D), s)
            else:
                L.call("amid_sas_wgrad_rows_sort_f32", ptr_array(dy), ptr_array(xx), 2, M, D, pl.splits,
                       ptr_array([pl.w_part[0].data_ptr(), pl.w_part[1].data_ptr()]), ptr_array([pl.b_part[0].data_ptr(), pl.b_part[1].data_ptr()]),
                       self._own_rows(pl), B, T, self._wgrad_mode(D), self._sort_plan_c(pl), s)
            self._enqueue_grad_tail(pl, live, seq)
            return
        L.call("amid_sas_wgrad_rows_f32", ptr_array(dy), ptr_array(xx), 2, M, D, pl.splits, ptr_array([pl.w_part[0].data_ptr(), pl.w_part[1].data_ptr()]),
               ptr_array([pl.b_part[0].data_ptr(), pl.b_part[1].data_ptr()]), self._own_rows(pl), B, T,
               self._wgrad_mode(D), s)
        if getattr(pl, "riding", False):
            L.call("amid_embed_bwd_sort_f32", (pl.dx0 if self.inc_bs else pl.dxg).data_ptr(), pl.tmq.data_ptr(), B, T, D, pl.pos_splits,
                   pl.dpos_part.data_ptr(), st, tr, SASREC_P_DROP, dom if live else None, self._sort_plan(pl), 5, s)
        elif live:
            L.call("amid_embed_bwd_rows_f32", (pl.dx0 if self.inc_bs else pl.dxg).data_ptr(), pl.tmq.data_ptr(), B, T, D, pl.pos_splits,
                   pl.dpos_part.data_ptr(), st, tr, SASREC_P_DROP, dom, s)
        else:
            L.call("amid_embed_bwd_f32", (pl.dx0 if self.inc_bs else pl.dxg).data_ptr(), pl.tmq.data_ptr(), B, T, D, pl.pos_splits,
                   pl.dpos_part.data_ptr(), st, tr, SASREC_P_DROP, s)
        if self.inc_bs:
            G = self.dense.grad
            head = (pl.dpos_part.data_ptr(), pl.pos_splits, pl.xg.data_ptr(), pl.dx0.data_ptr(), pl.inc_gate.data_ptr(), pl.inc_S.data_ptr(),
                    pl.inc_sw.data_ptr(), self._pp("inc_d{d}.trans_nn.weight"), self._pp("inc_d{d}.trans_nn.bias"),
                    self._pp("inc_d{d}.trans_bs.weight"), B, shp.T, D)
            outs = (pl.inc_dZ.data_ptr(), pl.inc_dS.data_ptr(), pl.inc_rows.data_ptr(), self._pp("inc_d{d}.trans_nn.weight", G),
                    self._pp("inc_d{d}.trans_nn.bias", G), self._pp("inc_d{d}.trans_bs.weight", G), self._pp("inc_d{d}.trans_bs.bias", G),
                    pl.dxg.data_ptr(), s)
            if getattr(pl, "inc_world", 1) > 1:
                ex = self._inc_exchange(pl)
                shard = (self.inc_bs, ex.rank * B)
                L.call("amid_inc_bwd_shard_f32", *head, *shard, 1, 1.0 / ex.world, *outs)
                self._coll(lambda: ex.all_reduce_dense(pl.inc_dZ))
                L.call("amid_inc_bwd_shard_f32", *head, *shard, 2, 1.0 / ex.world, *outs)
            else:
                L.call("amid_inc_bwd_f32", *head, *outs)
        self._enqueue_grad_tail(pl, live, seq)

    def _enqueue_grad_tail(self, pl: SasrecPlan, live: bool = False, seq: bool = False) -> None:
        L, s, shp = lib(), self.s, pl.shape
        if getattr(self, "_sort_owed", False):
            self.ev_idx.record(self.stream)
            self.enqueue_sort(pl)
        self.join_sort()
        blk = (pl.red_blk_s if seq else getattr(pl, "red_blk_v", None) if live else None) or pl.red_blk
        ent, n_ent, ent_max = ((pl.red_entries_s, pl.red_n_s, pl.red_max_s) if seq else (pl.red_entries_v, pl.red_n_v, pl.red_max_v) if live
                               else (pl.red_entries, pl.red_n, pl.red_max))
        pk = getattr(self, "_tail_pack", None)
        pl.spans_done = False
        if getattr(pl, "tail2", False) and not getattr(self, "_in_train_step", False):
            ent_t, n_ent_t, blk_t = self._tail2_table(pl)
            fp = self.dense
            head = (pl.dxg.data_ptr(), pl.pos_sorted.data_ptr(), pl.seg_off.data_ptr(), pl.seg_of.data_ptr(), pl.n_compact, self.D,
                    pl.seg_ws.data_ptr())
            mid = (ent_t.data_ptr(), n_ent_t, blk_t[0].data_ptr(), blk_t[1], pl.live.data_ptr(), shp.B, shp.Tenc,
                   fp.ptr("sac1.pos_emb.weight", fp.grad), fp.ptr("sac2.pos_emb.weight", fp.grad))
            if self.FUSED_OPT:
                left_lo = fp.slots["predictModule.fc.0.weight"][0]
                dense = (fp.grad.data_ptr(), fp.numel, left_lo, fp.numel, pl.uniq_ids.data_ptr(), pl.n_uniq.data_ptr(), pl.n_compact)
                if pk is not None:
                    from .dist import packed_rows
                    send, umax, with_dense = pk
                    id_rows, rows = packed_rows(umax, self.D)
                    L.call("amid_grad_tail_live_dp1_f32", *head, send.data_ptr() + 4 * id_rows * self.D, *mid, *dense, umax, self.n_rows,
                           send.data_ptr(), send.data_ptr() + 4 * rows * self.D if with_dense else None, pl.err.data_ptr(),
                           pl.tail_ticket.data_ptr(), s)
                else:
                    L.call("amid_grad_tail_live_dp1_f32", *head, pl.uniq_grad.data_ptr(), *mid, *dense, 0, 0, None, None, None,
                           pl.tail_ticket.data_ptr(), s)
            elif pk is not None:
                from .dist import packed_rows
                send, umax, with_dense = pk
                id_rows, rows = packed_rows(umax, self.D)
                L.call("amid_grad_tail_live_dp_f32", *head, send.data_ptr() + 4 * id_rows * self.D, *mid, pl.uniq_ids.data_ptr(),
                       pl.n_uniq.data_ptr(), umax, self.n_rows, send.data_ptr(), self.dense.grad.data_ptr() if with_dense else None,
                       send.data_ptr() + 4 * rows * self.D if with_dense else None, self.dense.numel if with_dense else 0,
                       pl.err.data_ptr(), s)
            else:
                L.call("amid_grad_tail_live_dp_f32", *head, pl.uniq_grad.data_ptr(), *mid, None, None, 0, 0, None, None, None, 0, None, s)
            pl.spans_done = True
            return
        pl.opt_done = False
        if getattr(pl, "tail2", False) and self.FUSED_OPT and self.table_m is not None and not self.dr:
            ent_t, n_ent_t, blk_t = self._tail2_table(pl)
            fp = self.dense
            left_lo = fp.slots["predictModule.fc.0.weight"][0]
            L.call("amid_grad_tail_opt_f32", pl.dxg.data_ptr(), pl.pos_sorted.data_ptr(), pl.seg_off.data_ptr(), pl.seg_of.data_ptr(), pl.n_compact,
                   self.D, pl.seg_ws.data_ptr(), pl.uniq_grad.data_ptr(), ent_t.data_ptr(), n_ent_t, blk_t[0].data_ptr(), blk_t[1],
                   pl.live.data_ptr(), shp.B, shp.Tenc, fp.ptr("sac1.pos_emb.weight", fp.grad), fp.ptr("sac2.pos_emb.weight", fp.grad),
                   fp.data.data_ptr(), fp.m.data_ptr(), fp.v.data_ptr(), fp.grad.data_ptr(), fp.numel, left_lo, fp.numel,
                   self.table.data_ptr(), self.table_m.data_ptr(), self.table_v.data_ptr(), self.table_last.data_ptr(), pl.uniq_ids.data_ptr(),
                   pl.n_uniq.data_ptr(), pl.n_compact, self.grad_scale, self.step_state.data_ptr(), pl.tail_ticket.data_ptr(), s)
            pl.opt_done = True
            return
        if getattr(pl, "tail2", False):
            ent_t, n_ent_t, blk_t = self._tail2_table(pl)
            fp = self.dense
            L.call("amid_grad_tail_live_f32", pl.dxg.data_ptr(), pl.pos_sorted.data_ptr(), pl.seg_off.data_ptr(), pl.seg_of.data_ptr(), pl.n_compact,
                   self.D, pl.seg_ws.data_ptr(), pl.uniq_grad.data_ptr(), ent_t.data_ptr(), n_ent_t, blk_t[0].data_ptr(), blk_t[1],
                   pl.live.data_ptr(), shp.B, shp.Tenc, fp.ptr("sac1.pos_emb.weight", fp.grad), fp.ptr("sac2.pos_emb.weight", fp.grad),
                   None, None, None, 0, 0, None, None, None, None, s)
            return
        if pk is not None:
            from .dist import packed_rows
            send, umax, with_dense = pk
            id_rows, rows = packed_rows(umax, self.D)
            L.call("amid_grad_tail_pack_f32", pl.dxg.data_ptr(), pl.pos_sorted.data_ptr(), pl.seg_off.data_ptr(), pl.seg_of.data_ptr(), self.n_sparse(pl),
                   self.D, pl.seg_ws.data_ptr(), send.data_ptr() + 4 * id_rows * self.D, ent.data_ptr(),
                   n_ent, ent_max, pl.uniq_ids.data_ptr(), pl.n_uniq.data_ptr(), umax,
                   self.n_rows, send.data_ptr(), self.dense.grad.data_ptr() if with_dense else None,
                   send.data_ptr() + 4 * rows * self.D if with_dense else None, self.dense.numel if with_dense else 0,
                   pl.err.data_ptr(), blk[0].data_ptr(), blk[1], s)
            return
        spans_later = bool(self.FUSED_SPANS and getattr(self, "_in_train_step", False) and self.D in (64, 128, 256))
# ... 441 lines not shown
```

include/amid_hip.h:

```cpp
#ifndef AMID_HIP_H
#define AMID_HIP_H

#ifdef __cplusplus
extern "C" {
#endif

#define AMID_OK 0
#define AMID_ERR_ARG (-1)
#define AMID_ERR_UNSUPPORTED (-2)
#define AMID_FLAG_INDEX_RANGE (1)
#define AMID_FLAG_UMAX_EXCEEDED (2)

int amid_version(void);
const char* amid_error_string(int code);
int amid_device_sync(void);

int amid_step_state_bytes(void);
int amid_step_state_pack(void* host_buf, unsigned long long seed, long long step, double lr, double beta1, double beta2, double eps);
int amid_step_begin(void* step_state, void* stream);

int amid_gather_rows_f32(const float* table, long long n_rows, int D, const void* idx, int idx_is_i64, long long n_idx,
                         float* out, int* err_flag, void* stream);
int amid_pack_indices(const long long* i_node, const long long* neg, const long long* seq_d1, const long long* seq_d2,
                      int B, int T, int n_neg, long long n_rows, int* idx_all, int* err_flag, void* step_state_to_bump, void* stream);
// ... 316 lines not shown
                         const unsigned char* tmq, float ln_eps, int B, int T, int D, int H, const int* live, const void* step_state,
                         int train, float p_drop, void* stream);
int amid_sas_seq_fwd_variant(int v);
int amid_sas_seq_fwd_bf16w_f32(int n_layers, const float* const* x_in, float* xout, const float* const* ln1_w, const float* const* ln1_b,
                               const float* const* w_in, const float* const* b_in, const float* const* w_o, const float* const* b_o,
                               const float* const* ln2_w, const float* const* ln2_b, const float* const* w1, const float* const* b1,
                               const float* const* w2, const float* const* b2, float* const* qn, float* const* q, float* const* k,
                               float* const* v, float* const* o, float* const* stats, float* const* r, float* const* y, float* const* h,
                               const unsigned char* tmq, float ln_eps, int B, int T, int D, int H, const int* live,
                               const void* step_state, int train, float p_drop, const void* w16, void* stream);
int amid_sas_weights_bf16(const float* const* src, int n, int D, int transposed, void* dst16, void* stream);
int amid_sas_weights_bf16_planes(const float* const* src, int n, int D, int transposed, int planes, void* dst16, void* stream);
int amid_sas_seq_fwd_split_f32(int n_layers, const float* const* x_in, float* xout, const float* const* ln1_w, const float* const* ln1_b,
                               const float* const* w_in, const float* const* b_in, const float* const* w_o, const float* const* b_o,
                               const float* const* ln2_w, const float* const* ln2_b, const float* const* w1, const float* const* b1,
                               const float* const* w2, const float* const* b2, float* const* qn, float* const* q, float* const* k,
                               float* const* v, float* const* o, float* const* stats, float* const* r, float* const* y, float* const* h,
                               const unsigned char* tmq, float ln_eps, int B, int T, int D, int H, const int* live,
                               const void* step_state, int train, float p_drop, const void* w16x3, void* stream);

int amid_sas_seq_bwd_supported(int B, int T, int D, int H);
int amid_sas_seq_bwd_variant(int v);
int amid_diag_variants(void);
int amid_sas_seq_bwd_f32(int n_layers, const float* dxo, const unsigned char* tmq, const float* const* h, const float* const* r,
                         const float* const* x, const float* const* q, const float* const* k, const float* const* v,
                         const float* const* o, const float* const* stats, const float* const* ln1_w, const float* const* ln2_w,
                         const float* const* wqT, const float* const* wkT, const float* const* wvT, const float* const* woT,
                         const float* const* w1T, const float* const* w2T, float ln_eps, int B, int T, int D, int H, const int* live,
                         const void* step_state, int train, float p_drop, float* const* dpre2, float* const* dpre1, float* const* dr,
                         float* d_o, float* const* dq, float* const* dk, float* const* dv, float* dx, float* const* ln1_part,
                         float* const* ln2_part, int mma_bf16, void* stream);

int amid_live_list_i32(const long long* domain, int B, int* live, void* stream);
int amid_pack_indices_live(const long long* i_node, const long long* neg, const long long* seq_d1, const long long* seq_d2, int B, int T,
                           int n_neg, long long n_rows, int* idx_all, int* err_flag, void* step_state_to_bump, const long long* domain,
                           int* live, void* stream);
int amid_pack_indices_pool_live(const long long* pool, long long pool_stride, int n_pool, long long phase, long long* in_pack,
                                int in_words, int B, int T, int n_neg, long long n_rows, int* idx_all, int* err_flag, void* step_state,
                                int* live, void* stream);
int amid_embed_bwd_sort_f32(float* dxg, const unsigned char* tmq, int B, int T, int D, int nsplit, float* dpos_part, const void* rng_state,
                            int train, float p_drop, const long long* row_domain, const void* sort_plan, int sort_phase, void* stream);
int amid_embed_fwd_live_f32(const float* table, const int* idx_all, const float* pos0, const float* pos1, int B, int T, int D,
                            int n_item_rows, float* xg, unsigned char* tmq, const void* rng_state, int train, float p_drop,
                            const int* live, void* stream);
int amid_embed_fwd_live_compact_f32(const float* table, const int* idx_all, const float* pos0, const float* pos1, int B, int T, int D,
                                    int n_item_rows, float* xg, unsigned char* tmq, const void* rng_state, int train, float p_drop,
                                    const int* live, int* idx_c, int* row_c, void* stream);
int amid_embed_fwd_replay_f32(const float* table, const float* m_tab, const float* v_tab, const int* last, const int* idx_all,
                              const float* pos0, const float* pos1, int B, int T, int D, int n_item_rows, float* xg,
                              unsigned char* tmq, const void* rng_state, int train, float p_drop, const int* live, int* idx_c,
                              int* row_c, const void* adam_state, const void* sort_plan, int sort_phase, void* stream);
int amid_embed_fwd_w16_f32(const float* table, const int* idx_all, const float* pos0, const float* pos1, int B, int T, int D, int n_item_rows,
                           float* xg, unsigned char* tmq, const void* rng_state, int train, float p_drop, const int* live, int* idx_c,
                           int* row_c, const float* const* w_src, int n_w, int w_planes, void* w16_dst, void* w16t_dst, void* stream);
int amid_attn_live_supported(int T, int D, int H, int causal);
int amid_attn_fwd_live_f32(const float* q, const float* k, const float* v, int B, int T, int D, int H, int causal, int layer,
                           const void* step_state, int train, float p_drop, float* o, float* stats, const int* live, void* stream);
int amid_attn_bwd_live_f32(const float* q, const float* k, const float* v, const float* o, const float* stats, const float* d_o, int B,
                           int T, int D, int H, int causal, int layer, const void* step_state, int train, float p_drop, float* dq,
                           float* dk, float* dv, const int* live, void* stream);
int amid_attn_long_live_supported(int T, int D, int H);
int amid_attn_fwd_long_live_infer_f32(const float* q, const float* k, const float* v, int B, int T, int D, int H, float* o, const int* live,
                                      void* stream);
int amid_head_fwd_bwd_own_f32(const float* x, const float* const* ln_w, const float* const* ln_b, const float* items, const float* w1,
                              const float* b1, const float* w2, const float* b2, const float* labels, const long long* domain_id, int B,
                              int T, int NI, int D, int hid, float eps, float* u, float* p1, float* p2, float* dp1, float* dp2,
                              float* loss_part, float* dx, float* ditems, float* ln_part, float* sc_part, const float* const* tr_src,
                              float* const* tr_dst, int n_tr, void* stream);

int amid_sas_strip_tile_rows(void);
int amid_sas_strip_qkv_fwd_f32(const float* x, const float* const* ln_w, const float* const* ln_b, const float* const* w_in,
                               const float* const* b_in, float ln_eps, int B, int T, int D, const int* live, float* qn, float* q, float* k,
                               float* v, void* stream);
int amid_sas_strip_oproj_ffn_fwd_f32(const float* o, const float* qn, const float* const* w_o, const float* const* b_o,
                                     const float* const* ln_w, const float* const* ln_b, const float* const* w1, const float* const* b1,
                                     const float* const* w2, const float* const* b2, const unsigned char* tmq, float ln_eps, int B, int T,
                                     int D, const int* live, int layer, const void* step_state, int train, float p_drop, float* r, float* y,
                                     float* h, float* xo, const float* const* nln_w, const float* const* nln_b, const float* const* nw_in,
                                     const float* const* nb_in, float* nqn, float* nq, float* nk, float* nv, void* stream);
int amid_sas_strip_infer_supported(int T, int D);
int amid_sas_strip_qkv_fwd_gather_infer_f32(const float* table, const int* idx_all, const float* pos0, const float* pos1,
                                            const float* const* ln_w, const float* const* ln_b, const float* const* w_in,
                                            const float* const* b_in, float ln_eps, int B, int T, int D, const int* live, unsigned char* tmq,
                                            float* qn, float* q, float* k, float* v, void* stream);
int amid_sas_strip_oproj_ffn_fwd_infer_f32(const float* o, const float* qn, const float* const* w_o, const float* const* b_o,
                                           const float* const* ln_w, const float* const* ln_b, const float* const* w1,
                                           const float* const* b1, const float* const* w2, const float* const* b2, const unsigned char* tmq,
                                           float ln_eps, int B, int T, int D, const int* live, float* xo, const float* const* nln_w,
                                           const float* const* nln_b, const float* const* nw_in, const float* const* nb_in, float* nqn,
                                           float* nq, float* nk, float* nv, void* stream);
int amid_sas_strip_ffn_bwd_f32(const float* dxo, const unsigned char* tmq, const float* h, const float* r, const float* const* ln_w,
                               const float* const* w1T, const float* const* w2T, const float* const* woT, float ln_eps, int B, int T, int D,
                               const int* live, int layer, const void* step_state, int train, float p_drop, float* dpre2, float* dpre1,
                               float* dr, float* d_o, float* ln_part, int mma_bf16, void* stream);
int amid_sas_strip_qkv_bwd_f32(const float* dq, const float* dk, const float* dv, const float* dr, const float* x, const float* const* ln_w,
                               const float* const* wqT, const float* const* wkT, const float* const* wvT, float ln_eps, int B, int T, int D,
                               const int* live, float* dx, float* ln_part, const unsigned char* tmq, const float* fh, const float* fr,
                               const float* const* fln_w, const float* const* fw1T, const float* const* fw2T, const float* const* fwoT,
                               int flayer, const void* step_state, int train, float p_drop, float* fdpre2, float* fdpre1, float* fdr,
                               float* fd_o, float* fln_part, int mma_bf16, void* stream);
int amid_sas_strip_ffn_bwd_sort_f32(const float* dxo, const unsigned char* tmq, const float* h, const float* r, const float* const* ln_w,
                               const float* const* w1T, const float* const* w2T, const float* const* woT, float ln_eps, int B, int T, int D,
                               const int* live, int layer, const void* step_state, int train, float p_drop, float* dpre2, float* dpre1,
                               float* dr, float* d_o, float* ln_part, const void* sort_plan, int sort_phase, int mma_bf16, void* stream);
int amid_sas_strip_qkv_bwd_sort_f32(const float* dq, const float* dk, const float* dv, const float* dr, const float* x, const float* const* ln_w,
                               const float* const* wqT, const float* const* wkT, const float* const* wvT, float ln_eps, int B, int T, int D,
                               const int* live, float* dx, float* ln_part, const unsigned char* tmq, const float* fh, const float* fr,
                               const float* const* fln_w, const float* const* fw1T, const float* const* fw2T, const float* const* fwoT,
                               int flayer, const void* step_state, int train, float p_drop, float* fdpre2, float* fdpre1, float* fdr,
                               float* fd_o, float* fln_part, const void* sort_plan, int sort_phase, int mma_bf16, void* stream);

int amid_embed_bwd_rows_f32(float* dxg, const unsigned char* tmq, int B, int T, int D, int nsplit, float* dpos_part, const void* rng_state,
                            int train, float p_drop, const long long* row_domain, void* stream);


int amid_bert_wgrad_rows_f32(const float* const* dy, const float* const* x, const int* ldy, const int* ldx, const int* out_ld,
                             const int* out_group, const int* out_col, int n_ent, int M, int splits, float* w_part, float* b_part,
                             const long long* row_domain, int B, int T, void* stream);


int amid_bert_wgrad_mode_f32(const float* const* dy, const float* const* x, const int* ldy, const int* ldx, const int* out_ld,
                             const int* out_group, const int* out_col, int n_ent, int M, int splits, float* w_part, float* b_part,
                             const long long* row_domain, int B, int T, int mode, void* stream);

int amid_bert_qkv_fwd_f32_rt4(const float* x, const float* const* ln_a, const float* const* ln_b, const float* const* w3x2,
                          const float* const* b3x2, int M, int rows_per_tile, float* y, float* q, float* k, float* v, void* stream);
int amid_bert_oproj_fwd_f32_rt4(const float* o, const float* x, const float* const* w, const float* const* b, int M, int rows_per_tile, int layer,
                            const void* step_state, int train, float p_drop, float* x1, void* stream);
int amid_bert_ffn1_fwd_f32_rt4(const float* x1, const float* const* ln_a, const float* const* ln_b, const float* const* w1, const float* const* b1,
                           int M, int rows_per_tile, int layer, const void* step_state, int train, float p_drop, float* y2, float* pre,
                           float* h, void* stream);
int amid_bert_ffn2_fwd_f32_rt4(const float* h, const float* x1, const float* const* w2, const float* const* b2, int M, int rows_per_tile, int layer,
                           const void* step_state, int train, float p_drop, float* x2, void* stream);
int amid_bert_ffn2_bwd_f32_rt4(const float* dx2, const float* pre, const float* const* w2T, int M, int rows_per_tile, int layer,
                           const void* step_state, int train, float p_drop, float* dz, float* dpre, void* stream);
int amid_bert_ffn1_bwd_f32_rt4(const float* dpre, const float* dx2, const float* x1, const float* const* ln_a, const float* const* w1T,
                           const float* const* woT, int M, int rows_per_tile, int layer, const void* step_state, int train, float p_drop,
                           float* dx1, float* dt, float* d_o, float* ln_part, void* stream);
int amid_bert_qkv_bwd_f32_rt4(const float* dq, const float* dk, const float* dv, const float* dx1, const float* x, const float* const* ln_a,
                          const float* const* wT3x2, int M, int rows_per_tile, float* dx, float* ln_part, void* stream);

int amid_step_head_f32(const long long* pool, long long pool_stride, int n_pool, long long phase, long long* in_pack, int in_words, int B, int T,
                       int n_neg, long long n_rows, int* idx_all, int* idx_c, int* row_c, int* live, int* err_flag, float* table, float* m,
                       float* v, int* last, int D, void* step_state, const void* sort_plan, void* stream);
int amid_sas_strip_qkv_bwd_emb_f32(const float* dq, const float* dk, const float* dv, const float* dr, const float* x, const float* const* ln_w,
                                   const float* const* wqT, const float* const* wkT, const float* const* wvT, float ln_eps, int B, int T, int D,
                                   const int* live, float* dx, float* ln_part, const unsigned char* emb_tmq, const void* step_state, int train,
                                   float emb_p_drop, const void* sort_plan, int sort_phase, int mma_bf16, void* stream);
int amid_sas_strip_ffn_bwd_px_f32(const float* dxo, const unsigned char* tmq, const float* h, const float* r, const float* const* ln_w,
                                  const float* const* w1T, const float* const* w2T, const float* const* woT, float ln_eps, int B, int T, int D,
                                  const int* live, int layer, const void* step_state, int train, float p_drop, float* dpre2, float* dpre1,
                                  float* dr, float* d_o, float* ln_part, const float* ln_stat, const void* sort_plan, int sort_phase,
                                  void* stream);
int amid_sas_wgrad_rows_sort_f32(const float* const* dy, const float* const* x, int n_layers, int M, int D, int splits, float* const* w_part,
                                 float* const* b_part, const long long* row_domain, int B, int T, int mma_bf16, const void* sort_plan,
                                 void* stream);
int amid_sas_seq_fwd_split_lnstat_f32(int n_layers, const float* const* x_in, float* xout, const float* const* ln1_w, const float* const* ln1_b,
                                      const float* const* w_in, const float* const* b_in, const float* const* w_o, const float* const* b_o,
                                      const float* const* ln2_w, const float* const* ln2_b, const float* const* w1, const float* const* b1,
                                      const float* const* w2, const float* const* b2, float* const* ln_stat, float* const* q, float* const* k,
                                      float* const* v, float* const* o, float* const* stats, float* const* r, float* const* h,
                                      const unsigned char* tmq, float ln_eps, int B, int T, int D, int H, const int* live,
                                      const void* step_state, int train, float p_drop, const void* w16x3, void* stream);
int amid_sas_seq_fwd_split_lnstat_head_f32(int n_layers, const float* const* x_in, float* xout, const float* const* ln1_w, const float* const* ln1_b,
                                           const float* const* w_in, const float* const* b_in, const float* const* w_o, const float* const* b_o,
                                           const float* const* ln2_w, const float* const* ln2_b, const float* const* w1, const float* const* b1,
                                           const float* const* w2, const float* const* b2, float* const* ln_stat, float* const* q,
                                           float* const* k, float* const* v, float* const* o, float* const* stats, float* const* r,
                                           float* const* h, const unsigned char* tmq, float ln_eps, int B, int T, int D, int H, const int* live,
                                           const void* step_state, int train, float p_drop, const void* w16x3,
                                           const float* const* last_ln_w, const float* const* last_ln_b, const float* items, const float* sw1,
                                           const float* sb1, const float* sw2, const float* sb2, const float* labels, const long long* domain_id,
                                           int NI, int hid, float* u, float* p1, float* p2, float* dp1, float* dp2, float* loss_part, float* dx,
                                           float* ditems, float* ln_part, float* hidg, void* stream);
int amid_sas_wgrad_rows_sort_ln_f32(const float* const* dy, const float* const* x, int n_layers, int M, int D, int splits, float* const* w_part,
                                    float* const* b_part, const long long* row_domain, int B, int T, int mma_bf16, const void* sort_plan,
                                    const float* const* ln_stat, const float* const* ln1_w, const float* const* ln1_b,
                                    const float* const* ln2_w, const float* const* ln2_b, void* stream);
int amid_grad_tail_live_f32(const float* grad_rows, const int* pos_sorted, const int* seg_off, const int* seg_of, int n_idx, int D,
                            void* workspace, float* uniq_grad, const void* entries_dev, int n_entries, const int* blk_off, int total_blocks,
                            const int* live, int B, int T, float* dpos0, float* dpos1, const float* hidg, const float* u,
                            const float* items, int NI, int hid, float* dW1, float* db1, float* dW2, float* db2, void* stream);
int amid_grad_tail_live_dp_f32(const float* grad_rows, const int* pos_sorted, const int* seg_off, const int* seg_of, int n_idx, int D,
                               void* workspace, float* uniq_grad, const void* entries_dev, int n_entries, const int* blk_off, int total_blocks,
                               const int* live, int B, int T, float* dpos0, float* dpos1, const int* uniq_ids, const int* n_uniq, int n_out,
                               int pad_id, int* out_ids, const float* dense_src, float* dense_dst, long long dense_n, int* err_flag,
                               void* stream);
long long amid_scorer_vec_floats(int NI, int hid);
int amid_sas_strip_qkv_bwd_sort_scorer_f32(const float* dq, const float* dk, const float* dv, const float* dr, const float* x,
                                           const float* const* ln_w, const float* const* wqT, const float* const* wkT,
                                           const float* const* wvT, float ln_eps, int B, int T, int D, const int* live, float* ln_part,
                                           const unsigned char* tmq, const float* fh, const float* fr, const float* const* fln_w,
                                           const float* const* fw1T, const float* const* fw2T, const float* const* fwoT, int flayer,
                                           const void* step_state, int train, float p_drop, float* fdpre2, float* fdpre1, float* fdr,
                                           float* fd_o, float* fln_part, const void* sort_plan, int sort_phase, int mma_bf16,
                                           const float* hidg, const float* u, const float* items, int NI, int hid, float* dW1, float* db1,
                                           float* dW2, float* db2, void* stream);
int amid_head_fwd_bwd_own_vec_f32(const float* x, const float* const* ln_w, const float* const* ln_b, const float* items, const float* w1,
                                  const float* b1, const float* w2, const float* b2, const float* labels, const long long* domain_id, int B,
                                  int T, int NI, int D, int hid, float eps, float* u, float* p1, float* p2, float* dp1, float* dp2,
                                  float* loss_part, float* dx, float* ditems, float* ln_part, float* hidg, const float* const* tr_src,
                                  float* const* tr_dst, int n_tr, void* stream);
int amid_grad_tail_nospans_f32(const float* grad_rows, const int* pos_sorted, const int* seg_off, const int* seg_of, int n_idx, int D,
                               void* workspace, float* uniq_grad, const void* entries_dev, int n_entries, int max_count, const int* blk_off,
                               int total_blocks, void* stream);
int amid_optimizer_step_spans_f32(float* p, float* m, float* v, const float* g, long long n, float* table, float* m_tab, float* v_tab, int* last,
                                  const int* uniq_ids, const int* n_uniq, int n_uniq_max, float* uniq_grad, int D, float grad_scale,
                                  const void* step_state, const int* seg_off, const int* seg_of, int n_sorted, const void* workspace,
                                  void* stream);

int amid_sas_seq_fwd_gather_head_f32(int n_layers, const float* const* x_in, float* xout, const float* const* ln1_w, const float* const* ln1_b,
                                     const float* const* w_in, const float* const* b_in, const float* const* w_o, const float* const* b_o,
                                     const float* const* ln2_w, const float* const* ln2_b, const float* const* w1, const float* const* b1,
                                     const float* const* w2, const float* const* b2, float* const* ln_stat, float* const* q, float* const* k,
                                     float* const* v, float* const* o, float* const* stats, float* const* r, float* const* h, unsigned char* tmq,
                                     float ln_eps, int B, int T, int D, int H, const int* live, void* step_state, int train, float p_drop,
                                     const void* w16x3, const float* const* last_ln_w, const float* const* last_ln_b, float* items,
                                     const float* sw1, const float* sb1, const float* sw2, const float* sb2, const float* labels,
                                     const long long* domain_id, int NI, int hid, float* u, float* p1, float* p2, float* dp1, float* dp2,
                                     float* loss_part, float* dx, float* ditems, float* ln_part, float* hidg, const float* table,
                                     const int* idx_all, const float* pos0, const float* pos1, void* stream);
int amid_sas_seq_fwd_gather_f32(int n_layers, const float* const* x_in, float* xout, const float* const* ln1_w, const float* const* ln1_b,
                                const float* const* w_in, const float* const* b_in, const float* const* w_o, const float* const* b_o,
                                const float* const* ln2_w, const float* const* ln2_b, const float* const* w1, const float* const* b1,
                                const float* const* w2, const float* const* b2, float* const* ln_stat, float* const* q, float* const* k,
                                float* const* v, float* const* o, float* const* stats, float* const* r, float* const* h, unsigned char* tmq,
                                float ln_eps, int B, int T, int D, int H, const int* live, void* step_state, int train, float p_drop,
                                const void* w16x3, float* items, int NI, const float* table, const int* idx_all, const float* pos0,
                                const float* pos1, void* stream);
int amid_sas_seq_fwd_gather_head_p1_f32(int n_layers, const float* const* x_in, float* xout, const float* const* ln1_w, const float* const* ln1_b,
                                     const float* const* w_in, const float* const* b_in, const float* const* w_o, const float* const* b_o,
                                     const float* const* ln2_w, const float* const* ln2_b, const float* const* w1, const float* const* b1,
                                     const float* const* w2, const float* const* b2, float* const* ln_stat, float* const* q, float* const* k,
                                     float* const* v, float* const* o, float* const* stats, float* const* r, float* const* h, unsigned char* tmq,
                                     float ln_eps, int B, int T, int D, int H, const int* live, void* step_state, int train, float p_drop,
                                     const void* w16x3, const float* const* last_ln_w, const float* const* last_ln_b, float* items,
                                     const float* sw1, const float* sb1, const float* sw2, const float* sb2, const float* labels,
                                     const long long* domain_id, int NI, int hid, float* u, float* p1, float* p2, float* dp1, float* dp2,
                                     float* loss_part, float* dx, float* ditems, float* ln_part, float* hidg, const float* table,
                                     const int* idx_all, const float* pos0, const float* pos1, void* stream);
int amid_sas_seq_fwd_gather_p1_f32(int n_layers, const float* const* x_in, float* xout, const float* const* ln1_w, const float* const* ln1_b,
                                const float* const* w_in, const float* const* b_in, const float* const* w_o, const float* const* b_o,
                                const float* const* ln2_w, const float* const* ln2_b, const float* const* w1, const float* const* b1,
                                const float* const* w2, const float* const* b2, float* const* ln_stat, float* const* q, float* const* k,
                                float* const* v, float* const* o, float* const* stats, float* const* r, float* const* h, unsigned char* tmq,
                                float ln_eps, int B, int T, int D, int H, const int* live, void* step_state, int train, float p_drop,
                                const void* w16x3, float* items, int NI, const float* table, const int* idx_all, const float* pos0,
                                const float* pos1, void* stream);

int amid_sas_seq_fwd_gather_infer_f32(int n_layers, float* xout, const float* const* ln1_w, const float* const* ln1_b, const float* const* w_in,
                                      const float* const* b_in, const float* const* w_o, const float* const* b_o, const float* const* ln2_w,
                                      const float* const* ln2_b, const float* const* w1, const float* const* b1, const float* const* w2,
                                      const float* const* b2, float ln_eps, int B, int T, int D, int H, const int* live, const void* w16x3,
                                      const float* table, const int* idx_all, const float* pos0, const float* pos1, void* stream);
int amid_step_head_w16_f32(const long long* pool, long long pool_stride, int n_pool, long long phase, long long* in_pack, int in_words, int B, int T,
                           int n_neg, long long n_rows, int* idx_all, int* idx_c, int* row_c, int* live, int* err_flag, float* table, float* m,
                           float* v, int* last, int D, void* step_state, const void* sort_plan, const float* const* w_src, int n_w, int w_planes,
                           void* w16_dst, void* w16t_dst, void* stream);

int amid_grad_tail_opt_f32(const float* grad_rows, const int* pos_sorted, const int* seg_off, const int* seg_of, int n_idx, int D,
                           void* workspace, float* uniq_grad, const void* entries_dev, int n_entries, const int* blk_off, int total_blocks,
                           const int* live, int B, int T, float* dpos0, float* dpos1, float* p, float* m, float* v, float* g, long long n,
                           long long left_lo, long long left_hi, float* table, float* m_tab, float* v_tab, int* last, const int* uniq_ids,
                           const int* n_uniq, int n_uniq_max, float grad_scale, const void* step_state, int* ticket, void* stream);

int amid_grad_tail_live_dp1_f32(const float* grad_rows, const int* pos_sorted, const int* seg_off, const int* seg_of, int n_idx, int D,
                                void* workspace, float* uniq_grad, const void* entries_dev, int n_entries, const int* blk_off, int total_blocks,
                                const int* live, int B, int T, float* dpos0, float* dpos1, float* g, long long n, long long left_lo,
                                long long left_hi, const int* uniq_ids, const int* n_uniq, int n_uniq_max, int n_out, int pad_id, int* out_ids,
                                float* dense_dst, int* err_flag, int* ticket, void* stream);

int amid_sas_seq_fwd_split_infer_f32(int n_layers, const float* x0, float* xout, const float* const* ln1_w, const float* const* ln1_b,
                                     const float* const* w_in, const float* const* b_in, const float* const* w_o, const float* const* b_o,
                                     const float* const* ln2_w, const float* const* ln2_b, const float* const* w1, const float* const* b1,
                                     const float* const* w2, const float* const* b2, const unsigned char* tmq, float ln_eps, int B, int T,
                                     int D, int H, const int* live, const void* w16x3, void* stream);
int amid_eval_head_f32(const float* x, const float* const* ln_w, const float* const* ln_b, const float* table, const int* ids,
                       const float* w1, const float* b1, const float* w2, const float* b2, const float* labels, const long long* domain_id,
                       int B, int T, int NI, int D, int hid, float eps, float fix_value, float* u, float* p, int* rank, int* rank_raw,
                       float* loss_part, void* stream);
int amid_eval_head_u_f32(const float* u_src, long long u_dom_stride, const float* table, const int* ids, const float* w1, const float* b1,
                         const float* w2, const float* b2, const float* labels, const long long* domain_id, int B, int NI, int D, int hid,
                         float fix_value, float* u, float* p, int* rank, int* rank_raw, float* loss_part, const float* itc_s,
                         const float* const* w_nn, const float* const* b_nn, const float* const* w_bs, const float* const* b_bs,
                         float threshold, float* gate, void* stream);

long long amid_full_rank_workspace_bytes(int B, int n_pool_d1, int n_pool_d2, int hid, int k);
int amid_full_rank_f32(const float* u, long long u_dom_stride, const long long* pos, const long long* domain_id, int B,
                       const long long* pool_d1, int n_pool_d1, const long long* pool_d2, int n_pool_d2, const long long* own_items,
                       const int* own_off, const int* rows, const float* table, long long n_rows, const float* w1, const float* b1,
                       const float* w2, const float* b2, int D, int hid, float fix_value, void* workspace, int* flags, int* rank,
                       int* rank_raw, float* scores, long long n_cols, void* stream);
int amid_topk_f32(const float* u, long long u_dom_stride, const long long* domain_id, int B, const long long* pool_d1, int n_pool_d1,
                  const long long* pool_d2, int n_pool_d2, const long long* own_items, const int* own_off, const int* rows,
                  const float* table, long long n_rows, const float* w1, const float* b1, const float* w2, const float* b2, int D,
                  int hid, int k, int exclude_history, void* workspace, int* flags, long long* ids, float* scores, void* stream);
int amid_topk_items_f32(int B, const long long* pool_d1, int n_pool_d1, const long long* pool_d2, int n_pool_d2, const float* table,
                        long long n_rows, const float* w1, int D, int hid, void* workspace, int* flags, void* stream);
int amid_topk_users_f32(const float* u, long long u_dom_stride, const long long* domain_id, int B, const long long* pool_d1, int n_pool_d1,
                        const long long* pool_d2, int n_pool_d2, const long long* own_items, const int* own_off, const int* rows,
                        const float* table, long long n_rows, const float* w1, const float* b1, const float* w2, const float* b2, int D,
                        int hid, int k, int exclude_history, void* workspace, int* flags, long long* ids, float* scores, void* stream);
int amid_own_from_seq_i64(const long long* seq_d1, const long long* seq_d2, const long long* domain_id, int B, int T, int* cnt,
                          long long* own, int* own_off, void* stream);

long long amid_neighbors_workspace_bytes(int Q, long long n_cand, int D, int k);
// ... 105 lines not shown
```

Baseline: 882,600 samples/s.

## Route strip backward kernels through split-row px path with LDS row-chain reductions

Adds a mode-4 path that sends the FFN and QKV strip backward launches (including the fused scorer and embedding-dropout variants) to a new px kernel family. That family splits each row across two wave groups and reduces LayerNorm row statistics through an LDS handoff chain. It also pre-scales the split-bf16 operands and uses its own weight ring with a mid-point sync. The engine turns the mode on for all three launches when D=128, p_drop=0.5 and the bf16x3 mode is active. The aim is more blocks per step and better overlap, at the cost of extra barriers, a larger LDS footprint and new numerical paths.

```diff
diff --git a/amid_amd/csrc/sasrec_strip.hip b/amid_amd/csrc/sasrec_strip.hip
--- a/amid_amd/csrc/sasrec_strip.hip
+++ b/amid_amd/csrc/sasrec_strip.hip
@@ -6,6 +6,7 @@
 #include "attention_mfma.h"
 #include "seq_bwd.h"
 #include "scorer_sum.h"
+#include "strip_px.h"
 #include <type_traits>
 
 namespace amid {
@@ -639,6 +640,8 @@
     int B = 0, T = 0, D = 0; const int* live = nullptr;
     const void* sort_plan = nullptr; int sort_phase = 0;
     int mma_bf16 = 0;
+    const float* ln_stat = nullptr;
+    const float* f_ln_stat = nullptr;
     void* stream = nullptr;
 };
 #define STRIP_BWD_LAUNCH(l) StripBwdLaunch l; l.B = B; l.T = T; l.D = D; l.live = live; l.mma_bf16 = mma_bf16; l.stream = stream
@@ -660,6 +663,7 @@
     SortRider rd;
     if (int e = make_rider(rd, l.sort_plan, l.sort_phase)) return e;
     if (rd.phase != 0 && rd.phase != 2) return AMID_ERR_UNSUPPORTED;
+    if (D == 128 && mma_bf16 == 4) return launch_ffn_bwd_px(a, l.ln_stat, sg, rd, l.stream);
     if (D == 128) return mma_bf16 == 3 ? launch_ffn_bwd<128, 3>(sg, rd, l.stream, a) : mma_bf16 ? launch_ffn_bwd<128, 1>(sg, rd, l.stream, a)
                                                                                           : launch_ffn_bwd<128, 0>(sg, rd, l.stream, a);
     if (D == 64) return launch_ffn_bwd<64, 0>(sg, rd, l.stream, a);
@@ -733,10 +737,11 @@
     if (rd.phase != 0 && rd.phase != (ffn ? 3 : 4)) return AMID_ERR_UNSUPPORTED;
     ScorerSum ss = {};
     if (c.scorer != nullptr) {
-        if (!(ffn && D == 128 && (mma_bf16 == 3 || mma_bf16 == 1))) return AMID_ERR_UNSUPPORTED;
+        if (!(ffn && D == 128 && (mma_bf16 == 3 || mma_bf16 == 1 || mma_bf16 == 4))) return AMID_ERR_UNSUPPORTED;
         ss = *c.scorer;
     }
     void* const st = l.stream;
+    if (D == 128 && mma_bf16 == 4) return launch_qkv_bwd_px(a, f, ffn, l.ln_stat, l.f_ln_stat, ss, sg, rd, st);
     if (D == 128 && mma_bf16 == 3) return ffn ? launch_qkv_bwd<128, true, 3>(sg, rd, st, a, f, ss) : launch_qkv_bwd<128, false, 3>(sg, rd, st, a, f, ss);
     if (D == 128 && mma_bf16) return ffn ? launch_qkv_bwd<128, true, 1>(sg, rd, st, a, f, ss) : launch_qkv_bwd<128, false, 1>(sg, rd, st, a, f, ss);
     if (D == 128) return ffn ? launch_qkv_bwd<128, true, 0>(sg, rd, st, a, f, ss) : launch_qkv_bwd<128, false, 0>(sg, rd, st, a, f, ss);
@@ -808,6 +813,29 @@
                                               float emb_p_drop, const void* sort_plan, int sort_phase, int mma_bf16, void* stream) {
     AMID_CHECK_ARG(emb_tmq != nullptr && dx != nullptr);
     STRIP_QKV_BWD_CALL(c); c.dx = dx; c.emb_tmq = emb_tmq; c.emb_p_drop = emb_p_drop; STRIP_BWD_LAUNCH(l); STRIP_BWD_RIDER(l);
+    return strip_qkv_bwd(c, l);
+}
+
+extern "C" int amid_sas_strip_qkv_bwd_px_f32(const float* dq, const float* dk, const float* dv, const float* dr, const float* x,
+                                             const float* const* ln_w, const float* const* wqT, const float* const* wkT, const float* const* wvT,
+                                             float ln_eps, int B, int T, int D, const int* live, float* dx, float* ln_part,
+                                             const unsigned char* tmq, const float* fh, const float* fr, const float* const* fln_w,
+                                             const float* const* fw1T, const float* const* fw2T, const float* const* fwoT, int flayer,
+                                             const void* step_state, int train, float p_drop, float* fdpre2, float* fdpre1, float* fdr,
+                                             float* fd_o, float* fln_part, const unsigned char* emb_tmq, float emb_p_drop, const float* ln_stat,
+                                             const float* f_ln_stat, const void* sort_plan, int sort_phase, const float* hidg, const float* u,
+                                             const float* items, int NI, int hid, float* dW1, float* db1, float* dW2, float* db2, void* stream) {
+    if (D != 128) return AMID_ERR_UNSUPPORTED;
+    const int mma_bf16 = 4;
+    ScorerSum ss = {};
+    if (hidg != nullptr) {
+        AMID_CHECK_ARG(fh != nullptr && u && items && NI > 0 && hid > 0 && dW1 && db1 && dW2 && db2);
+        AMID_CHECK_ARG(((((unsigned long long)dW1) | ((unsigned long long)u) | ((unsigned long long)items)) & 15) == 0);
+        ss = scorer_sum_args(hidg, u, items, B, NI, D, hid, dW1, db1, dW2, db2);
+    }
+    STRIP_QKV_BWD_CALL(c); STRIP_QKV_BWD_FFN(c); c.dx = dx; c.emb_tmq = emb_tmq; c.emb_p_drop = emb_p_drop;
+    if (hidg != nullptr) c.scorer = &ss;
+    STRIP_BWD_LAUNCH(l); STRIP_BWD_RIDER(l); l.ln_stat = ln_stat; l.f_ln_stat = f_ln_stat;
     return strip_qkv_bwd(c, l);
 }
 #undef AMID_FFN_BWD_CALL
diff --git a/amid_amd/csrc/sasrec_strip_px.hip b/amid_amd/csrc/sasrec_strip_px.hip
--- a/amid_amd/csrc/sasrec_strip_px.hip
+++ b/amid_amd/csrc/sasrec_strip_px.hip
@@ -6,12 +6,15 @@
 #include "seq_bwd.h"
 #include "seqn_parts.h"
 #include "sort_phases.h"
+#include "scorer_sum.h"
+#include "strip_px.h"
 
 namespace amid {
 
 constexpr int PXB_WPS = 4, PXB_NS = 2, PXB_NW = PXB_WPS * PXB_NS, PXB_THREADS = 64 * PXB_NW;
-template <int D> constexpr size_t pxb_lds_floats() {
-    return (size_t)3 * (D * D / 2) + (size_t)PXB_WPS * XpStrip<D>::FLOATS + 2 * PXB_NW * 16 + (size_t)PXB_WPS * 2 * D;
+constexpr int PXB_STAT_STRIP = 2 * 64 + 2 * 16, PXB_STAT = PXB_WPS * PXB_STAT_STRIP;
+template <int D> constexpr size_t pxb_lds_floats(int chains = 1) {
+    return (size_t)3 * (D * D / 2) + (size_t)PXB_WPS * XpStrip<D>::FLOATS + PXB_STAT + (size_t)chains * PXB_WPS * 2 * D;
 }
 
 struct PxbRow { unsigned off_own, phys; int local; bool ok; };
@@ -32,21 +35,23 @@
     return r;
 }
 
-template <int NCT>
-__device__ __forceinline__ void pxb_row_sums(float* __restrict__ stat, int si, int part, float s1, float s2, float& t1, float& t2) {
-    const int m = lane_id() & 15, gq = lane_id() >> 4;
-    s1 = row_sum4(s1); s2 = row_sum4(s2);
-    if (gq == 0) {
-        lds_st1(stat + (si * PXB_NS + part) * 16 + m, s1);
-        lds_st1(stat + (PXB_NW + si * PXB_NS + part) * 16 + m, s2);
-    }
+template <class Add>
+__device__ __forceinline__ void pxb_row_chain(float* __restrict__ stat, int si, int part, float& a, float& b, const Add& add) {
+    typedef __attribute__((address_space(3))) float lf;
+    float* ls = stat + si * PXB_STAT_STRIP;
+    float* rs = ls + 2 * 64;
+    const int lane = lane_id(), m = lane & 15;
+    a = 0.f; b = 0.f;
+    if (part == 0) { add(a, b); lds_st1(ls + lane, a); lds_st1(ls + 64 + lane, b); }
     lds_barrier();
-    t1 = 0.f; t2 = 0.f;
-#pragma unroll
-    for (int p = 0; p < PXB_NS; ++p) {
-        t1 += *(__attribute__((address_space(3))) float*)(stat + (si * PXB_NS + p) * 16 + m);
-        t2 += *(__attribute__((address_space(3))) float*)(stat + (PXB_NW + si * PXB_NS + p) * 16 + m);
-    }
+    if (part != 0) {
+        a = *(lf*)(ls + lane); b = *(lf*)(ls + 64 + lane);
+        add(a, b);
+        a = row_sum4(a); b = row_sum4(b);
+        if (lane < 16) { lds_st1(rs + m, a); lds_st1(rs + 16 + m, b); }
+    }
+    lds_barrier();
+    if (part == 0) { a = *(lf*)(rs + m); b = *(lf*)(rs + 16 + m); }
 }
 
 template <int D, int NCT>
@@ -70,77 +75,33 @@
         part[e] = (scratch[e] + scratch[2 * D + e]) + (scratch[4 * D + e] + scratch[6 * D + e]);
 }
 
-template <int D, int NCT, class Ring>
-__device__ __forceinline__ void pxb_ffn_bwd_chain(const StripFfnBwdArgs& a, const float* __restrict__ ln_stat, const StripGeom& sg, Ring& ring,
-                                                  const PxbRow& row, int g, int si, int part, int c0, PartRegs<NCT>& DZ, float* __restrict__ xps,
-                                                  float* __restrict__ stat, float* __restrict__ lnsc, const unsigned short* __restrict__ wnext) {
-    const int lane = lane_id(), gq = lane >> 4;
-    const GBuf gp2(a.dpre2, sg.act_bytes), gp1(a.dpre1, sg.act_bytes), gdr(a.dr, sg.act_bytes), gdo(a.d_o, sg.act_bytes);
-    PartRegs<NCT> P, Hs, Rs, gam;
-    part_load<NCT>(Hs, GBuf(a.h, sg.act_bytes), row.off_own);
-    part_load<NCT>(Rs, GBuf(a.r, sg.act_bytes), row.off_own);
-    part_cols<NCT>(gam, a.ln_w[g], c0);
-    float mean = 0.f, rstd = 0.f;
-    if (ln_stat != nullptr && row.ok) { mean = ln_stat[(long long)row.phys * 4 + 2]; rstd = ln_stat[(long long)row.phys * 4 + 3]; }
-    if (a.tmq != nullptr) {
-        const GBuf gtm(a.tmq, sg.tm_bytes);
-        const unsigned tbase = row.ok ? row.phys * (unsigned)(D / 4) + (unsigned)c0 * 4u : STRIP_OOB;
-        const int sh = 8 * gq;
+template <int D, int NCT>
+__device__ __forceinline__ void pxb_ln_bwd(PartRegs<NCT>& DR, const PartRegs<NCT>& dbet, const PartRegs<NCT>& X, const PartRegs<NCT>& gam, bool have_stat,
+                                           float mean, float& rstd, float eps, float* __restrict__ stat, int si, int part, PartRegs<NCT>& dgam,
+                                           const f32x4 (*addend)[NCT] = nullptr, PartRegs<NCT>* uout = nullptr) {
+    if (!have_stat) {
+        float tot, qt, dummy;
+        pxb_row_chain(stat, si, part, tot, dummy, [&](float& s, float&) {
+#pragma unroll
+            for (int c = 0; c < NCT; ++c) s += (X.v[c][0] + X.v[c][1]) + (X.v[c][2] + X.v[c][3]);
+        });
+        mean = tot * (1.0f / D);
+        pxb_row_chain(stat, si, part, qt, dummy, [&](float& q, float&) {
+#pragma unroll
+            for (int c = 0; c < NCT; ++c)
+#pragma unroll
+                for (int r = 0; r < 4; ++r) { const float d = X.v[c][r] - mean; q = fmaf(d, d, q); }
+        });
+        rstd = 1.0f / sqrtf(qt * (1.0f / D) + eps);
+    }
+    float t1, t2;
+    pxb_row_chain(stat, si, part, t1, t2, [&](float& s1, float& s2) {
 #pragma unroll
         for (int c = 0; c < NCT; ++c) {
-            const unsigned bits = (unsigned)__builtin_amdgcn_raw_buffer_load_b32(gtm.r, (int)(tbase + 4 * c), 0, 0) >> sh;
-            DZ.v[c][0] = (bits & 1u) ? 0.f : DZ.v[c][0];
-            DZ.v[c][1] = (bits & 2u) ? 0.f : DZ.v[c][1];
-            DZ.v[c][2] = (bits & 4u) ? 0.f : DZ.v[c][2];
-            DZ.v[c][3] = (bits & 8u) ? 0.f : DZ.v[c][3];
-        }
-    }
-    P = DZ;
-    if (a.train) {
-        const uint4 rr2 = rng_call(a.st->seed, (unsigned long long)row.local * D >> 7, site_id(g, a.layer, SITE_FFN2), (unsigned)a.st->step);
-        part_dropout<NCT>(P, rr2, c0, a.spec, a.scale, (row.local * D) & 127);
-    }
-    xp_write<NCT>(xps, c0, P);
-    f32x4 acc[NCT];
-    {
-        ring.next();
-        seqn_product_xp<D, NCT>(acc, xps, ring, (const unsigned short*)a.w1T[g], c0, [&](int ct, int j) { part_spread<NCT>(gp2, row.off_own, P, ct, j, 1); });
-#pragma unroll
-        for (int c = 0; c < NCT; ++c)
-#pragma unroll
-            for (int r = 0; r < 4; ++r) P.v[c][r] = Hs.v[c][r] > 0.f ? acc[c][r] * a.scale : 0.f;
-    }
-    lds_barrier();
-    xp_write<NCT>(xps, c0, P);
-    PartRegs<NCT> DR, dgam, dbet;
-    {
-        ring.next();
-        seqn_product_xp<D, NCT>(acc, xps, ring, (const unsigned short*)a.woT[g], c0, [&](int ct, int j) { part_spread<NCT>(gp1, row.off_own, P, ct, j, 1); });
-        if (ln_stat == nullptr) {
-            float sm = 0.f;
-#pragma unroll
-            for (int c = 0; c < NCT; ++c) sm += (Rs.v[c][0] + Rs.v[c][1]) + (Rs.v[c][2] + Rs.v[c][3]);
-            float tot, dummy;
-            pxb_row_sums<NCT>(stat, si, part, sm, 0.f, tot, dummy);
-            mean = tot * (1.0f / D);
-            float q = 0.f;
-#pragma unroll
-            for (int c = 0; c < NCT; ++c)
-#pragma unroll
-                for (int r = 0; r < 4; ++r) { const float d = Rs.v[c][r] - mean; q = fmaf(d, d, q); }
-            lds_barrier();
-            float qt;
-            pxb_row_sums<NCT>(stat, si, part, q, 0.f, qt, dummy);
-            rstd = 1.0f / sqrtf(qt * (1.0f / D) + a.ln_eps);
-            lds_barrier();
-        }
-        float s1 = 0.f, s2 = 0.f;
-#pragma unroll
-        for (int c = 0; c < NCT; ++c) {
 #pragma unroll
             for (int r = 0; r < 4; ++r) {
-                const float dy = acc[c][r] + DZ.v[c][r];
-                const float xh = (Rs.v[c][r] - mean) * rstd;
+                const float dy = dbet.v[c][r];
+                const float xh = (X.v[c][r] - mean) * rstd;
                 float gy = gam.v[c][r] * dy;
                 asm volatile("" : "+v"(gy));
                 s1 += gy;
@@ -148,31 +109,266 @@
                 float dg = dy * xh;
                 asm volatile("" : "+v"(dg));
                 dgam.v[c][r] = dg;
-                dbet.v[c][r] = dy;
                 DR.v[c][r] = gy;
             }
         }
-        float t1, t2;
-        pxb_row_sums<NCT>(stat, si, part, s1, s2, t1, t2);
-        const float c1 = t1 * (1.0f / D), c2 = t2 * (1.0f / D);
+    });
+    const float c1 = t1 * (1.0f / D), c2 = t2 * (1.0f / D);
+    {
+#pragma clang fp contract(off)
 #pragma unroll
         for (int c = 0; c < NCT; ++c)
 #pragma unroll
             for (int r = 0; r < 4; ++r) {
-                const float xh = (Rs.v[c][r] - mean) * rstd;
-                DR.v[c][r] = rstd * (DR.v[c][r] - c1 - xh * c2);
+                const float xh = (X.v[c][r] - mean) * rstd;
+                const float u = __builtin_fmaf(-xh, c2, DR.v[c][r] - c1);
+                if (uout != nullptr) uout->v[c][r] = u;
+                DR.v[c][r] = addend != nullptr ? __builtin_fmaf(rstd, u, (*addend)[c][r]) : rstd * u;
             }
     }
-    xp_write<NCT>(xps, c0, DR);
+}
+
+template <int NCT>
+__device__ __forceinline__ void xp_write_scaled(float* __restrict__ xps, int c0, const PartRegs<NCT>& u, float k) {
+#pragma clang fp contract(off)
+    const int lane = lane_id();
+    auto split = [&](float ua, float ub) {
+        WgSplit2 s;
+        s.hi = wg_pack2(k * ua, k * ub);
+        const float a1 = __builtin_fmaf(k, ua, -__uint_as_float(s.hi << 16)), b1 = __builtin_fmaf(k, ub, -__uint_as_float(s.hi & 0xffff0000u));
+        s.mid = wg_pack2(a1, b1);
+        const float a2 = a1 - __uint_as_float(s.mid << 16), b2 = b1 - __uint_as_float(s.mid & 0xffff0000u);
+        s.lo = wg_pack2(a2, b2);
+        return s;
+    };
+#pragma unroll
+    for (int e = 0; e < NCT / 2; ++e) {
+        const int st = c0 / 2 + e;
+        const WgSplit2 p0 = split(u.v[2 * e][0], u.v[2 * e][1]), p1 = split(u.v[2 * e][2], u.v[2 * e][3]);
+        const WgSplit2 p2 = split(u.v[2 * e + 1][0], u.v[2 * e + 1][1]), p3 = split(u.v[2 * e + 1][2], u.v[2 * e + 1][3]);
+        lds_st4(xps + ((st * 3 + 0) * 64 + lane) * 4, __builtin_bit_cast(f32x4, amid_v4u{p0.hi, p1.hi, p2.hi, p3.hi}));
+        lds_st4(xps + ((st * 3 + 1) * 64 + lane) * 4, __builtin_bit_cast(f32x4, amid_v4u{p0.mid, p1.mid, p2.mid, p3.mid}));
+        lds_st4(xps + ((st * 3 + 2) * 64 + lane) * 4, __builtin_bit_cast(f32x4, amid_v4u{p0.lo, p1.lo, p2.lo, p3.lo}));
+    }
+}
+
+template <int D, int NW> struct PxbRing : SeqRing3<D, NW> {
+    using Base = SeqRing3<D, NW>;
+    __device__ __forceinline__ explicit PxbRing(float* lds) : Base(lds) {}
+    __device__ __forceinline__ void next() {
+        w_ring_wait();
+        __syncthreads();
+        if (!this->hi_ready) this->plane(this->hslot(), this->cur);
+    }
+    __device__ __forceinline__ void mid_sync() {
+        w_ring_wait();
+        __syncthreads();
+        this->plane(this->mslot(), this->nxt + (size_t)D * D);
+        this->plane(this->lslot(), this->nxt + (size_t)2 * D * D);
+        this->cur = this->nxt; this->hi_ready = false;
+    }
+};
+
+template <int D, int NCT, class Ring>
+__device__ __forceinline__ void pxb_mma_xp(f32x4 (&acc)[NCT], const float* __restrict__ xps, Ring& ring, int c0) {
+    constexpr int KS = D / 32, NSTEP = KS * NCT, CT_BYTES = 16 * (D / 2) * 4, PLANE_BYTES = Ring::SLAB * 4;
+    constexpr int PD1 = FRAG_AHEAD_2, PD2 = FRAG_AHEAD_1;
+    static_assert(PD1 < NSTEP && PD2 < NSTEP && 2 * PD1 + 2 < 16, "read-ahead against the step count and the lgkmcnt field");
+    const int lane = lane_id();
+    const int i = lane & 15, g = lane >> 4;
+    auto mma = [&](const f32x4& wf, const f32x4& a16, const f32x4& c) {
+        return __builtin_amdgcn_mfma_f32_16x16x32_bf16(__builtin_bit_cast(seqn_bf16x8, wf), __builtin_bit_cast(seqn_bf16x8, a16), c, 0, 0, 0);
+    };
+    unsigned fo[KS];
+#pragma unroll
+    for (int s = 0; s < KS; ++s) fo[s] = (unsigned)((((c0 * 16 + i) * (D / 2)) + 4 * ((4 * s + g) ^ i)) * 4);
+    const unsigned xa = lds_offset(xps) + (unsigned)lane * 16u;
+    const unsigned mbase = lds_offset(ring.mslot());
+    static_assert(CT_BYTES * (NCT - 1) + PLANE_BYTES < 65536, "the lo plane is reached through the offset field");
+    const unsigned hbase = mbase + 2u * PLANE_BYTES;
+    {
+        f32x4 wm[PD1 + 1], wl[PD1 + 1], ah[KS], am[KS];
+        static_for<KS>([&](auto S) {
+            constexpr int s = decltype(S)::value;
+            lds_frag_issue<(s * 3 + 0) * 1024>(ah[s], xa);
+            lds_frag_issue<(s * 3 + 1) * 1024>(am[s], xa);
+        });
+        auto issue = [&](auto U) {
+            constexpr int u = decltype(U)::value, c = u / KS, s = u % KS, k = u % (PD1 + 1);
+            lds_frag_issue<c * CT_BYTES>(wm[k], mbase + fo[s]);
+            lds_frag_issue<c * CT_BYTES + PLANE_BYTES>(wl[k], mbase + fo[s]);
+        };
+        static_for<PD1>(issue);
+        static_for<NSTEP>([&](auto T) {
+            constexpr int t = decltype(T)::value, c = t / KS, s = t % KS, k = t % (PD1 + 1);
+            if constexpr (t + PD1 < NSTEP) issue(std::integral_constant<int, t + PD1>{});
+            constexpr int last = t + PD1 < NSTEP ? t + PD1 : NSTEP - 1;
+            asm volatile("s_waitcnt lgkmcnt(%4)" : "+v"(wm[k]), "+v"(wl[k]), "+v"(ah[s]), "+v"(am[s]) : "n"(2 * (last - t)));
+            acc[c] = mma(wm[k], am[s], acc[c]); acc[c] = mma(wl[k], ah[s], acc[c]); acc[c] = mma(wm[k], ah[s], acc[c]);
+        });
+    }
+    ring.mid_sync();
+    {
+        f32x4 wf[PD2 + 1], ah[KS], am[KS], al[KS];
+        static_for<KS>([&](auto S) {
+            constexpr int s = decltype(S)::value;
+            lds_frag_issue<(s * 3 + 0) * 1024>(ah[s], xa);
+            lds_frag_issue<(s * 3 + 1) * 1024>(am[s], xa);
+            lds_frag_issue<(s * 3 + 2) * 1024>(al[s], xa);
+        });
+        auto issue = [&](auto U) {
+            constexpr int u = decltype(U)::value, c = u / KS, s = u % KS;
+            lds_frag_issue<c * CT_BYTES>(wf[u % (PD2 + 1)], hbase + fo[s]);
+        };
+        static_for<PD2>(issue);
+        static_for<NSTEP>([&](auto T) {
+            constexpr int t = decltype(T)::value, c = t / KS, s = t % KS, k = t % (PD2 + 1);
+            if constexpr (t + PD2 < NSTEP) issue(std::integral_constant<int, t + PD2>{});
+            constexpr int last = t + PD2 < NSTEP ? t + PD2 : NSTEP - 1;
+            asm volatile("s_waitcnt lgkmcnt(%4)" : "+v"(wf[k]), "+v"(ah[s]), "+v"(am[s]), "+v"(al[s]) : "n"(last - t));
+            acc[c] = mma(wf[k], al[s], acc[c]); acc[c] = mma(wf[k], am[s], acc[c]); acc[c] = mma(wf[k], ah[s], acc[c]);
+        });
+    }
+}
+
+template <int D, int NCT, bool ZERO = true, class Ring, class Stores>
+__device__ __forceinline__ void pxb_product(f32x4 (&acc)[NCT], const float* __restrict__ xps, Ring& ring, const unsigned short* __restrict__ wn16, int c0,
+                                            const Stores& stores) {
+    if constexpr (ZERO) {
+#pragma unroll
+        for (int c = 0; c < NCT; ++c) acc[c] = f32x4{0.f, 0.f, 0.f, 0.f};
+    }
+    ring.begin(wn16);
+#pragma unroll
+    for (int ct = 0; ct < NCT; ++ct) { stores(ct, 1); stores(ct, 3); }
+    pxb_mma_xp<D, NCT, Ring>(acc, xps, ring, c0);
+}
+
+template <int D, int NCT>
+__device__ __forceinline__ void pxb_tm_load(unsigned (&bits)[NCT], const unsigned char* __restrict__ tmq, const StripGeom& sg, const PxbRow& row, int c0) {
+    const GBuf gtm(tmq, sg.tm_bytes);
+    const unsigned tbase = row.ok ? row.phys * (unsigned)(D / 4) + (unsigned)c0 * 4u : STRIP_OOB;
+    const int sh = 8 * (lane_id() >> 4);
+#pragma unroll
+    for (int c = 0; c < NCT; ++c) bits[c] = (unsigned)__builtin_amdgcn_raw_buffer_load_b32(gtm.r, (int)(tbase + 4 * c), 0, 0) >> sh;
+}
+template <int NCT>
+__device__ __forceinline__ void pxb_tm_apply(PartRegs<NCT>& x, const unsigned (&bits)[NCT]) {
+#pragma unroll
+    for (int c = 0; c < NCT; ++c) {
+        x.v[c][0] = (bits[c] & 1u) ? 0.f : x.v[c][0];
+        x.v[c][1] = (bits[c] & 2u) ? 0.f : x.v[c][1];
+        x.v[c][2] = (bits[c] & 4u) ? 0.f : x.v[c][2];
+        x.v[c][3] = (bits[c] & 8u) ? 0.f : x.v[c][3];
+    }
+}
+
+template <int NCT> struct PxbFfnPre { PartRegs<NCT> Hs, gam; unsigned tm[NCT]; float mean, rstd; };
+template <int D, int NCT>
+__device__ __forceinline__ void pxb_ffn_prefetch(PxbFfnPre<NCT>& p, const StripFfnBwdArgs& a, const float* __restrict__ ln_stat, const StripGeom& sg,
+                                                 const PxbRow& row, int g, int c0) {
+    part_load<NCT>(p.Hs, GBuf(a.h, sg.act_bytes), row.off_own);
+    if (a.tmq != nullptr) pxb_tm_load<D, NCT>(p.tm, a.tmq, sg, row, c0);
+    part_cols<NCT>(p.gam, a.ln_w[g], c0);
+    p.mean = 0.f; p.rstd = 0.f;
+    if (ln_stat != nullptr && row.ok) { p.mean = ln_stat[(long long)row.phys * 4 + 2]; p.rstd = ln_stat[(long long)row.phys * 4 + 3]; }
+}
+
+template <int D, int NCT, class Ring>
+__device__ __forceinline__ void pxb_ffn_bwd_chain(const StripFfnBwdArgs& a, const float* __restrict__ ln_stat, const StripGeom& sg, Ring& ring,
+                                                  const PxbRow& row, int g, int si, int part, int c0, PartRegs<NCT>& DZ, PxbFfnPre<NCT>& pre,
+                                                  float* __restrict__ xps, float* __restrict__ stat, float* __restrict__ lnsc,
+                                                  const unsigned short* __restrict__ wnext) {
+    const GBuf gp2(a.dpre2, sg.act_bytes), gp1(a.dpre1, sg.act_bytes), gdr(a.dr, sg.act_bytes), gdo(a.d_o, sg.act_bytes);
+    PartRegs<NCT> P, Rs;
+    PartRegs<NCT>& Hs = pre.Hs;
+    PartRegs<NCT>& gam = pre.gam;
+    float mean = pre.mean, rstd = pre.rstd;
+    if (a.tmq != nullptr) pxb_tm_apply<NCT>(DZ, pre.tm);
+    P = DZ;
+    if (a.train) {
+        const uint4 rr2 = rng_call(a.st->seed, (unsigned long long)row.local * D >> 7, site_id(g, a.layer, SITE_FFN2), (unsigned)a.st->step);
+        part_dropout<NCT>(P, rr2, c0, a.spec, a.scale, (row.local * D) & 127);
+    }
+    xp_write<NCT>(xps, c0, P);
+    f32x4 acc[NCT];
     {
         ring.next();
-        seqn_product_xp<D, NCT>(acc, xps, ring, wnext, c0, [&](int ct, int j) { part_spread<NCT>(gdr, row.off_own, DR, ct, j, 1); });
+        part_load<NCT>(Rs, GBuf(a.r, sg.act_bytes), row.off_own);
+        pxb_product<D, NCT>(acc, xps, ring, (const unsigned short*)a.w1T[g], c0, [&](int ct, int j) { part_spread<NCT>(gp2, row.off_own, P, ct, j, 1); });
+#pragma unroll
+        for (int c = 0; c < NCT; ++c)
+#pragma unroll
+            for (int r = 0; r < 4; ++r) P.v[c][r] = Hs.v[c][r] > 0.f ? acc[c][r] * a.scale : 0.f;
+    }
+    lds_barrier();
+    xp_write<NCT>(xps, c0, P);
+    PartRegs<NCT> DR, U, dgam, dbet;
+    {
+        ring.next();
+        pxb_product<D, NCT>(acc, xps, ring, (const unsigned short*)a.woT[g], c0, [&](int ct, int j) { part_spread<NCT>(gp1, row.off_own, P, ct, j, 1); });
+#pragma unroll
+        for (int c = 0; c < NCT; ++c) dbet.v[c] = acc[c] + DZ.v[c];
+        pxb_ln_bwd<D, NCT>(DR, dbet, Rs, gam, ln_stat != nullptr, mean, rstd, a.ln_eps, stat, si, part, dgam, nullptr, &U);
+        pxb_ln_partials<D, NCT>(lnsc, si, c0, dgam, dbet);
+    }
+    xp_write_scaled<NCT>(xps, c0, U, rstd);
+    {
+        ring.next();
+        pxb_product<D, NCT>(acc, xps, ring, wnext, c0, [&](int ct, int j) { part_spread<NCT>(gdr, row.off_own, DR, ct, j, 1); });
 #pragma unroll
         for (int c = 0; c < NCT; ++c) P.v[c] = acc[c];
         part_store<NCT>(gdo, row.off_own, P);
     }
-    pxb_ln_partials<D, NCT>(lnsc, si, c0, dgam, dbet);
-}
+}
+
+template <int D, int NCT, class Ring, class Hook>
+__device__ __forceinline__ void pxb_qkv_bwd_chain(const StripQkvBwdArgs& a, const float* __restrict__ ln_stat, const StripGeom& sg, Ring& ring,
+                                                  const PxbRow& row, int g, int si, int part, int c0, const PartRegs<NCT>& Dk, const PartRegs<NCT>& Dv,
+                                                  PartRegs<NCT>& DX, float* __restrict__ xps, float* __restrict__ stat, float* __restrict__ lnsc,
+                                                  const unsigned short* __restrict__ wnext, const Hook& before_last) {
+    PartRegs<NCT> Dq, Drs, Xs, gam;
+    f32x4 acc_kv[NCT], acc[NCT];
+    const auto none = [](int, int) {};
+    xp_write<NCT>(xps, c0, Dk);
+    {
+        ring.next();
+        part_load<NCT>(Dq, GBuf(a.dq, sg.act_bytes), row.off_own);
+        pxb_product<D, NCT>(acc_kv, xps, ring, (const unsigned short*)a.wvT[g], c0, none);
+    }
+    lds_barrier();
+    xp_write<NCT>(xps, c0, Dv);
+    float mean = 0.f, rstd = 0.f;
+    {
+        ring.next();
+        part_load<NCT>(Drs, GBuf(a.dr, sg.act_bytes), row.off_own);
+        part_load<NCT>(Xs, GBuf(a.x, sg.act_bytes), row.off_own);
+        part_cols<NCT>(gam, a.ln_w[g], c0);
+        if (ln_stat != nullptr && row.ok) { mean = ln_stat[(long long)row.phys * 4]; rstd = ln_stat[(long long)row.phys * 4 + 1]; }
+        pxb_product<D, NCT, false>(acc_kv, xps, ring, (const unsigned short*)a.wqT[g], c0, none);
+    }
+    lds_barrier();
+    xp_write<NCT>(xps, c0, Dq);
+    PartRegs<NCT> dgam;
+    {
+        ring.next();
+        before_last();
+        pxb_product<D, NCT>(acc, xps, ring, wnext, c0, none);
+#pragma unroll
+        for (int c = 0; c < NCT; ++c) Drs.v[c] += acc[c];
+        pxb_ln_bwd<D, NCT>(DX, Drs, Xs, gam, ln_stat != nullptr, mean, rstd, a.ln_eps, stat, si, part, dgam, &acc_kv);
+    }
+    pxb_ln_partials<D, NCT>(lnsc, si, c0, dgam, Drs);
+}
+
+struct PxbWave { int part, si, c0; };
+template <int NCT> __device__ __forceinline__ PxbWave pxb_wave() {
+    const int w = wave_id();
+    return PxbWave{w / PXB_WPS, w % PXB_WPS, (w / PXB_WPS) * NCT};
+}
+template <int D> __device__ __forceinline__ float* pxb_xps(float* smem, int si) { return smem + 3 * SeqRing3<D, PXB_NW>::SLAB + si * XpStrip<D>::FLOATS; }
+template <int D> __device__ __forceinline__ float* pxb_stat(float* smem) { return smem + 3 * SeqRing3<D, PXB_NW>::SLAB + PXB_WPS * XpStrip<D>::FLOATS; }
+template <int D> __device__ __forceinline__ float* pxb_lnsc(float* smem, int which) { return pxb_stat<D>(smem) + PXB_STAT + which * PXB_WPS * 2 * D; }
 
 template <int D, int RIDER>
 __global__ __launch_bounds__(PXB_THREADS) void strip_ffn_bwd_px_kernel(const StripFfnBwdArgs a, const float* __restrict__ ln_stat, const StripGeom sg,
@@ -184,22 +380,115 @@
         if (bid < rd.plan.nblk) { if (threadIdx.x < SORT_THREADS) sort_phase_ct<RIDER>(rd.plan, bid, smem); return; }
         bid -= rd.plan.nblk;
     }
-    const int w = wave_id(), part = w / PXB_WPS, si = w % PXB_WPS, c0 = part * NCT;
-    const int g = strip_domain(bid);
-    SeqRing3<D, PXB_NW> ring(smem);
+    const PxbWave wv = pxb_wave<NCT>();
+    const StripTile t = strip_tile(sg, bid);
+    if (!t.live) { zero_slot<D>(a.ln_part, t.slot); return; }
+    const int g = t.g;
+    const PxbRow row = pxb_row<D>(sg, t, wv.si, wv.c0);
+    PartRegs<NCT> DZ;
+    PxbFfnPre<NCT> pre;
+    part_load<NCT>(DZ, GBuf(a.dxo, sg.act_bytes), row.off_own);
+    pxb_ffn_prefetch<D, NCT>(pre, a, ln_stat, sg, row, g, wv.c0);
+    PxbRing<D, PXB_NW> ring(smem);
     ring.first((const unsigned short*)a.w2T[g]);
-    const StripTile t = strip_tile(sg, bid);
-    if (!t.live) { zero_slot<D>(a.ln_part, t.slot); w_ring_wait(); return; }
-    float* const xps = smem + 3 * SeqRing3<D, PXB_NW>::SLAB + si * XpStrip<D>::FLOATS;
-    float* const stat = smem + 3 * SeqRing3<D, PXB_NW>::SLAB + PXB_WPS * XpStrip<D>::FLOATS;
-    float* const lnsc = stat + 2 * PXB_NW * 16;
-    const PxbRow row = pxb_row<D>(sg, t, si, c0);
-    PartRegs<NCT> DZ;
-    part_load<NCT>(DZ, GBuf(a.dxo, sg.act_bytes), row.off_own);
-    pxb_ffn_bwd_chain<D, NCT>(a, ln_stat, sg, ring, row, g, si, part, c0, DZ, xps, stat, lnsc, (const unsigned short*)a.woT[g]);
+    float* const lnsc = pxb_lnsc<D>(smem, 0);
+    pxb_ffn_bwd_chain<D, NCT>(a, ln_stat, sg, ring, row, g, wv.si, wv.part, wv.c0, DZ, pre, pxb_xps<D>(smem, wv.si), pxb_stat<D>(smem), lnsc,
+                              (const unsigned short*)a.woT[g]);
     w_ring_wait();
     __syncthreads();
     pxb_ln_partials_out<D>(lnsc, a.ln_part + (long long)t.slot * 2 * D);
+}
+
+template <int D, bool FFN, int RIDER>
+__global__ __launch_bounds__(PXB_THREADS) void strip_qkv_bwd_px_kernel(const StripQkvBwdArgs a, const StripFfnBwdArgs f, const float* __restrict__ ln_stat,
+                                                                       const float* __restrict__ f_ln_stat, const ScorerSum ss, const StripGeom sg,
+                                                                       const SortRider rd) {
+    extern __shared__ __attribute__((aligned(16))) float smem[];
+    constexpr int NCT = D / 16 / PXB_NS;
+    int bid = blockIdx.x;
+    if constexpr (RIDER != 0 && FFN) {
+        if (ss.front) {
+            if (bid < ss.nblk) { if (threadIdx.x < STRIP_THREADS) scorer_sum_block(ss, bid, (scorer_lds_f4*)smem); return; }
+            bid -= ss.nblk;
+        } else {
+            const int first = (int)gridDim.x - ss.nblk;
+            if (bid >= first) { if (threadIdx.x < STRIP_THREADS) scorer_sum_block(ss, bid - first, (scorer_lds_f4*)smem); return; }
+        }
+    }
+    if constexpr (RIDER > 0) {
+        if (bid < rd.plan.nblk) { if (threadIdx.x < SORT_THREADS) sort_phase_ct<RIDER>(rd.plan, bid, smem); return; }
+        bid -= rd.plan.nblk;
+    }
+    const PxbWave wv = pxb_wave<NCT>();
+    const StripTile t = strip_tile(sg, bid);
+    if (!t.live) {
+        zero_slot<D>(a.ln_part, t.slot);
+        if constexpr (FFN) zero_slot<D>(f.ln_part, t.slot);
+        return;
+    }
+    const int g = t.g;
+    const PxbRow row = pxb_row<D>(sg, t, wv.si, wv.c0);
+    PartRegs<NCT> Dk, Dv, DX;
+    part_load<NCT>(Dk, GBuf(a.dk, sg.act_bytes), row.off_own);
+    part_load<NCT>(Dv, GBuf(a.dv, sg.act_bytes), row.off_own);
+    PxbRing<D, PXB_NW> ring(smem);
+    ring.first((const unsigned short*)a.wkT[g]);
+    float* const xps = pxb_xps<D>(smem, wv.si);
+    float* const stat = pxb_stat<D>(smem);
+    if constexpr (FFN) {
+        PxbFfnPre<NCT> pre;
+        pxb_qkv_bwd_chain<D, NCT>(a, ln_stat, sg, ring, row, g, wv.si, wv.part, wv.c0, Dk, Dv, DX, xps, stat, pxb_lnsc<D>(smem, 0),
+                                  (const unsigned short*)f.w2T[g], [&]() { pxb_ffn_prefetch<D, NCT>(pre, f, f_ln_stat, sg, row, g, wv.c0); });
+        pxb_ffn_bwd_chain<D, NCT>(f, f_ln_stat, sg, ring, row, g, wv.si, wv.part, wv.c0, DX, pre, xps, stat, pxb_lnsc<D>(smem, 1),
+                                  (const unsigned short*)f.woT[g]);
+    } else {
+        const bool emb = a.emb_tmq != nullptr;
+        unsigned etm[NCT];
+        pxb_qkv_bwd_chain<D, NCT>(a, ln_stat, sg, ring, row, g, wv.si, wv.part, wv.c0, Dk, Dv, DX, xps, stat, pxb_lnsc<D>(smem, 0),
+                                  (const unsigned short*)a.wkT[g], [&]() { if (emb) pxb_tm_load<D, NCT>(etm, a.emb_tmq, sg, row, wv.c0); });
+        if (emb) {
+            if (a.emb_train) {
+                const uint4 rr = rng_call(a.emb_st->seed, (unsigned long long)row.local * D >> 7, site_id(g, 0, SITE_EMB), (unsigned)a.emb_st->step);
+                part_dropout<NCT>(DX, rr, wv.c0, a.emb_spec, a.emb_scale, (row.local * D) & 127);
+            }
+            pxb_tm_apply<NCT>(DX, etm);
+        }
+        part_store<NCT>(GBuf(a.dx, sg.act_bytes), row.off_own, DX);
+    }
+    w_ring_wait();
+    __syncthreads();
+    pxb_ln_partials_out<D>(pxb_lnsc<D>(smem, 0), a.ln_part + (long long)t.slot * 2 * D);
+    if constexpr (FFN) pxb_ln_partials_out<D>(pxb_lnsc<D>(smem, 1), f.ln_part + (long long)t.slot * 2 * D);
+}
+
+using namespace amid_strip_host;
+
+static bool pxb_dropout_ok(int train, unsigned spec) { return !train || spec_bits(spec) == 1; }
+
+int launch_ffn_bwd_px(const StripFfnBwdArgs& a, const float* ln_stat, const StripGeom& sg, const SortRider& rd, void* stream) {
+    if (!pxb_dropout_ok(a.train, a.spec)) return AMID_ERR_UNSUPPORTED;
+    if (rd.phase != 0 && rd.phase != 2) return AMID_ERR_UNSUPPORTED;
+    constexpr size_t lds = pxb_lds_floats<128>() * sizeof(float);
+    static_assert(lds >= sizeof(SortScatterLds<OS_BINS_MAX>), "the rider's scatter fits the head of the allocation");
+    if (rd.phase != 0) return launch_lds<strip_ffn_bwd_px_kernel<128, 2>>(2 * sg.tpg + rd.plan.nblk, PXB_THREADS, lds, stream, a, ln_stat, sg, rd);
+    return launch_lds<strip_ffn_bwd_px_kernel<128, 0>>(2 * sg.tpg, PXB_THREADS, lds, stream, a, ln_stat, sg, rd);
+}
+
+int launch_qkv_bwd_px(const StripQkvBwdArgs& a, const StripFfnBwdArgs& f, bool ffn, const float* ln_stat, const float* f_ln_stat, const ScorerSum& ss,
+                      const StripGeom& sg, const SortRider& rd, void* stream) {
+    if (!pxb_dropout_ok(a.emb_train, a.emb_spec) || (ffn && !pxb_dropout_ok(f.train, f.spec))) return AMID_ERR_UNSUPPORTED;
+    if (rd.phase != 0 && rd.phase != (ffn ? 3 : 4)) return AMID_ERR_UNSUPPORTED;
+    if (ss.nblk > 0 && !ffn) return AMID_ERR_UNSUPPORTED;
+    constexpr size_t lds1 = pxb_lds_floats<128>(1) * sizeof(float), lds2 = pxb_lds_floats<128>(2) * sizeof(float);
+    static_assert(lds2 <= 160 * 1024, "the fused launch's second LayerNorm scratch fits the CU's LDS");
+    static_assert(lds1 >= sizeof(SortScatterLds<OS_BINS_MAX>) && lds1 >= 8 * 33 * 16, "a rider's scratch fits the head of the allocation");
+    const int tiles = 2 * sg.tpg, sortb = rider_blocks_host(rd);
+    if (ffn) {
+        if (rd.phase) return launch_lds<strip_qkv_bwd_px_kernel<128, true, 3>>(tiles + sortb + ss.nblk, PXB_THREADS, lds2, stream, a, f, ln_stat, f_ln_stat, ss, sg, rd);
+        return launch_lds<strip_qkv_bwd_px_kernel<128, true, -1>>(tiles + ss.nblk, PXB_THREADS, lds2, stream, a, f, ln_stat, f_ln_stat, ss, sg, rd);
+    }
+    if (rd.phase) return launch_lds<strip_qkv_bwd_px_kernel<128, false, 4>>(tiles + sortb, PXB_THREADS, lds1, stream, a, f, ln_stat, f_ln_stat, ss, sg, rd);
+    return launch_lds<strip_qkv_bwd_px_kernel<128, false, 0>>(tiles, PXB_THREADS, lds1, stream, a, f, ln_stat, f_ln_stat, ss, sg, rd);
 }
 
 }
@@ -227,9 +516,6 @@
         rd.plan = *(const SortPlan*)sort_plan;
         rd.phase = sort_phase;
     }
-    constexpr size_t lds = pxb_lds_floats<128>() * sizeof(float);
-    static_assert(lds >= sizeof(SortScatterLds<OS_BINS_MAX>), "the rider's scatter fits the head of the allocation");
-    if (rd.phase != 0) return launch_lds<strip_ffn_bwd_px_kernel<128, 2>>(2 * sg.tpg + rd.plan.nblk, PXB_THREADS, lds, stream, a, ln_stat, sg, rd);
-    return launch_lds<strip_ffn_bwd_px_kernel<128, 0>>(2 * sg.tpg, PXB_THREADS, lds, stream, a, ln_stat, sg, rd);
+    return launch_ffn_bwd_px(a, ln_stat, sg, rd, stream);
 }
 #undef AMID_FFN_BWD_CALL
diff --git a/amid_amd/csrc/strip_px.h b/amid_amd/csrc/strip_px.h
--- /dev/null
+++ b/amid_amd/csrc/strip_px.h
@@ -0,0 +1,12 @@
+#pragma once
+#include "seq_bwd.h"
+#include "sort_phases.h"
+#include "scorer_sum.h"
+
+namespace amid {
+
+int launch_ffn_bwd_px(const StripFfnBwdArgs& a, const float* ln_stat, const StripGeom& sg, const SortRider& rd, void* stream);
+int launch_qkv_bwd_px(const StripQkvBwdArgs& a, const StripFfnBwdArgs& f, bool ffn, const float* ln_stat, const float* f_ln_stat, const ScorerSum& ss,
+                      const StripGeom& sg, const SortRider& rd, void* stream);
+
+}
diff --git a/amid_amd/engine.py b/amid_amd/engine.py
--- a/amid_amd/engine.py
+++ b/amid_amd/engine.py
@@ -234,6 +234,10 @@
     _bf16_bwd = False
     _p3_bwd = False
     BWD_SPLIT = True
+    STRIP_NSPLIT = 7
+
+    def _strip_mode(self, bf: int, launch: int) -> int:
+        return 4 if bf == 3 and self.D == 128 and SASREC_P_DROP == 0.5 and (int(self.STRIP_NSPLIT) >> launch) & 1 else bf
 
     def enqueue_prepare(self, pl: SasrecPlan, sparse: bool, bump_step: bool = False, defer_sort: bool = False) -> None:
         L, s, shp = lib(), self.s, pl.shape
@@ -932,7 +936,7 @@
             ride = lambda ph: (plan_addr, ph) if riding else ()
             L.call(f"amid_sas_strip_ffn_bwd{sfx}_f32", pl.dxbuf.data_ptr(), tm, h1, r1, lnw1, w1T1, w2T1, woT1, SASREC_LN_EPS, B, T, D, lv, 1, st, tr,
                    SASREC_P_DROP, pl.dpre2[1].data_ptr(), pl.dpre1[1].data_ptr(), pl.dr[1].data_ptr(), pl.d_o.data_ptr(), ln2p[1].data_ptr(),
-                   *ride(2), bf, s)
+                   *ride(2), self._strip_mode(bf, 0), s)
             attn_bwd(1)
             if t2:
                 mid = ("amid_sas_strip_qkv_bwd_sort_scorer_f32", dict(sort_plan=plan_addr, sort_phase=3)) if riding else ("amid_sas_strip_qkv_bwd_scorer_f32", {})
@@ -942,23 +946,23 @@
                              wvT=self._wT(1, 2), ln_eps=SASREC_LN_EPS, B=B, T=T, D=D, live=lv, ln_part=ln1p[1].data_ptr(), tmq=tm, fh=h0, fr=r0,
                              fln_w=lnw0, fw1T=w1T0, fw2T=w2T0, fwoT=woT0, flayer=0, step_state=st, train=tr, p_drop=SASREC_P_DROP,
                              fdpre2=pl.dpre2[0].data_ptr(), fdpre1=pl.dpre1[0].data_ptr(), fdr=pl.dr[0].data_ptr(), fd_o=pl.d_o.data_ptr(),
-                             fln_part=ln2p[0].data_ptr(), mma_bf16=bf, hidg=self._hidg(pl).data_ptr(),
+                             fln_part=ln2p[0].data_ptr(), mma_bf16=self._strip_mode(bf, 1), hidg=self._hidg(pl).data_ptr(),
                              u=pl.u.data_ptr(), items=items, NI=NI, hid=self.hid, stream=s)
             else:
                 L.call(f"amid_sas_strip_qkv_bwd{sfx}_f32", pl.dq_l[1].data_ptr(), pl.dk_l[1].data_ptr(), pl.dv_l[1].data_ptr(), pl.dr[1].data_ptr(),
                        pl.x[1].data_ptr(), self._pp("sac{d}.attention_layernorms.1.weight"), self._wT(1, 0), self._wT(1, 1), self._wT(1, 2),
                        SASREC_LN_EPS, B, T, D, lv, None, ln1p[1].data_ptr(), tm, h0, r0, lnw0, w1T0, w2T0, woT0, 0, st, tr, SASREC_P_DROP,
-                       pl.dpre2[0].data_ptr(), pl.dpre1[0].data_ptr(), pl.dr[0].data_ptr(), pl.d_o.data_ptr(), ln2p[0].data_ptr(), *ride(3), bf, s)
+                       pl.dpre2[0].data_ptr(), pl.dpre1[0].data_ptr(), pl.dr[0].data_ptr(), pl.d_o.data_ptr(), ln2p[0].data_ptr(), *ride(3), self._strip_mode(bf, 1), s)
             attn_bwd(0)
             if t2:
                 L.call("amid_sas_strip_qkv_bwd_emb_f32", pl.dq_l[0].data_ptr(), pl.dk_l[0].data_ptr(), pl.dv_l[0].data_ptr(), pl.dr[0].data_ptr(),
                        pl.x[0].data_ptr(), self._pp("sac{d}.attention_layernorms.0.weight"), self._wT(0, 0), self._wT(0, 1), self._wT(0, 2),
-                       SASREC_LN_EPS, B, T, D, lv, dx_in, ln1p[0].data_ptr(), pl.tmq.data_ptr(), st, tr, SASREC_P_DROP, plan_addr, 4 if riding else 0, bf, s)
+                       SASREC_LN_EPS, B, T, D, lv, dx_in, ln1p[0].data_ptr(), pl.tmq.data_ptr(), st, tr, SASREC_P_DROP, plan_addr, 4 if riding else 0, self._strip_mode(bf, 2), s)
             else:
                 L.call(f"amid_sas_strip_qkv_bwd{sfx}_f32", pl.dq_l[0].data_ptr(), pl.dk_l[0].data_ptr(), pl.dv_l[0].data_ptr(), pl.dr[0].data_ptr(),
                        pl.x[0].data_ptr(), self._pp("sac{d}.attention_layernorms.0.weight"), self._wT(0, 0), self._wT(0, 1), self._wT(0, 2),
                        SASREC_LN_EPS, B, T, D, lv, dx_in, ln1p[0].data_ptr(), None, None, None, None, None, None, None, 0, None, 0, 0.0, None,
-                       None, None, None, None, *ride(4), bf, s)
+                       None, None, None, None, *ride(4), self._strip_mode(bf, 2), s)
         else:
             rows, suf, rpt = ("_rows", pl.rt_suffix_v, pl.rpt_v) if live else ("", pl.rt_suffix, pl.rpt)
             ln1p, ln2p = (pl.ln1_part_v, pl.ln2_part_v) if live else (pl.ln1_part, pl.ln2_part)
diff --git a/include/amid_hip.h b/include/amid_hip.h
--- a/include/amid_hip.h
+++ b/include/amid_hip.h
@@ -492,6 +492,14 @@
                                   const int* live, int layer, const void* step_state, int train, float p_drop, float* dpre2, float* dpre1,
                                   float* dr, float* d_o, float* ln_part, const float* ln_stat, const void* sort_plan, int sort_phase,
                                   void* stream);
+int amid_sas_strip_qkv_bwd_px_f32(const float* dq, const float* dk, const float* dv, const float* dr, const float* x, const float* const* ln_w,
+                                  const float* const* wqT, const float* const* wkT, const float* const* wvT, float ln_eps, int B, int T, int D,
+                                  const int* live, float* dx, float* ln_part, const unsigned char* tmq, const float* fh, const float* fr,
+                                  const float* const* fln_w, const float* const* fw1T, const float* const* fw2T, const float* const* fwoT,
+                                  int flayer, const void* step_state, int train, float p_drop, float* fdpre2, float* fdpre1, float* fdr,
+                                  float* fd_o, float* fln_part, const unsigned char* emb_tmq, float emb_p_drop, const float* ln_stat,
+                                  const float* f_ln_stat, const void* sort_plan, int sort_phase, const float* hidg, const float* u,
+                                  const float* items, int NI, int hid, float* dW1, float* db1, float* dW2, float* db2, void* stream);
 int amid_sas_wgrad_rows_sort_f32(const float* const* dy, const float* const* x, int n_layers, int M, int D, int splits, float* const* w_part,
                                  float* const* b_part, const long long* row_domain, int B, int T, int mma_bf16, const void* sort_plan,
                                  void* stream);
```

After: 895,900 samples/s (median of 6 runs). +1.5%, better.
